# ambicuity/Distributed-LLM-Training-and-Inference-System

Measured on AMD Instinct MI355X. Metric: tokens/sec (node) GPT-7B train, higher is better.
Workload: dtype bf16; 1 GPU; model=gpt-7b, global_batch=16, seq_len=2048, parallelism=dp1, micro_batch=16, grad_accum=1, activation_checkpoint=none, layout=planner

## Files before the change

### llmctl/config/knobs.py

```python

from __future__ import annotations

import contextlib
import dataclasses
import os
from dataclasses import dataclass, fields
from typing import Any, Dict, Iterator, Optional

ENV = "LLMCTL_KNOBS"


@dataclass(frozen=True)
class PerfKnobs:
    gemm64: bool = True
    gemm64_config: int = 304
    fwd64: str = "auto"
    dgrad64: str = "fused"
    wgrad_kernel: bool = True
    swiglu_bwd: str = "side"
    dgrad_transpose: bool = True
    wt_side_stream: bool = True
    fused_fwd: bool = False
    rope_inplace: bool = True
    fused_rope_attn: bool = True
    moe_pad: bool = True
    overlap_optimizer: bool = False
    gemm_tuning: bool = True
    fa_split: int = -1
    fa_prio: int = 1
    fa_nw: int = 4
    dkv: int = 2
    dkv_nwg: int = 0
    async_tp: bool = True
    async_tp_save_full: bool = False
    cp_zigzag: bool = True
    decode_fused: bool = True
    decode_splits: int = 0
    decode_v3: int = 1
    skinny_gemm: str = "auto"
    prefill_swiglu: bool = True
    prefill_fa: bool = True
    prefill_norm_fold: bool = True
    mixed_steps: bool = True
    custom_ar: bool = True
    tp_graphs: bool = True
    async_decode: bool = True
    tp_fused_decode: bool = True

    def as_dict(self) -> Dict[str, Any]:
        return dataclasses.asdict(self)


NATIVE = ("fa_split", "fa_prio", "fa_nw", "dkv", "dkv_nwg", "decode_splits", "decode_v3")
_FIELDS = {f.name: f for f in fields(PerfKnobs)}


def _coerce(name: str, value: Any) -> Any:
    if name not in _FIELDS:
        raise KeyError(f"unknown performance knob {name!r} (known: {', '.join(sorted(_FIELDS))})")
    typ = _FIELDS[name].type
    if typ in ("bool", bool):
        if isinstance(value, str):
            v = value.strip().lower()
            if v not in ("1", "0", "true", "false", "on", "off", "yes", "no"):
                raise ValueError(f"knob {name}: expected a boolean, got {value!r}")
            return v in ("1", "true", "on", "yes")
        return bool(value)
    if typ in ("int", int):
        return int(value)
    return str(value)


def parse_env(spec: Optional[str]) -> Dict[str, Any]:
    out: Dict[str, Any] = {}
    for part in (spec or "").split(","):
        part = part.strip()
        if not part:
            continue
        if "=" not in part:
            raise ValueError(f"{ENV}: expected name=value, got {part!r}")
        k, v = part.split("=", 1)
        out[k.strip()] = _coerce(k.strip(), v.strip())
    return out


_RETIRED_ENV = ("LLMCTL_SIDE_DGRAD", "LLMCTL_DECODE_ATTN_QKV", "LLMCTL_GEMM64_CONFIG", "LLMCTL_SKINNY")
_warned: set = set()


def _warn_retired_env() -> None:
    import warnings

    names = [f"LLMCTL_{n.upper()}" for n in _FIELDS] + list(_RETIRED_ENV)
    for n in names:
        if n in os.environ and n not in _warned:
            _warned.add(n)
            warnings.warn(f"{n} is no longer read (performance switches are knobs now): set "
                          f"{ENV}=\"{n[7:].lower()}=<value>\" or the [perf] config table instead", stacklevel=3)


def resolve(overrides: Optional[Dict[str, Any]] = None, env: bool = True) -> PerfKnobs:
    _warn_retired_env()
    kw = {k: _coerce(k, v) for k, v in (overrides or {}).items()}
    if env:
        kw.update(parse_env(os.environ.get(ENV)))
    return PerfKnobs(**kw)


_ACTIVE: PerfKnobs = resolve()


def knobs() -> PerfKnobs:
    return _ACTIVE


def push_native(k: Optional[PerfKnobs] = None) -> bool:
    k = k or _ACTIVE
    try:
        from llmctl.ops import _lib

        if not _lib.loaded():
            return False
        import torch

        for name in NATIVE:
            torch.ops.llmctl.set_knob(name, int(getattr(k, name)))
        return True
    except Exception:
        return False


def apply(k: PerfKnobs) -> PerfKnobs:
    global _ACTIVE
    _ACTIVE = k
    push_native(k)
    return k


def use(k: PerfKnobs) -> PerfKnobs:
    if k is not _ACTIVE:
        apply(k)
    return k


def with_env(k: PerfKnobs) -> PerfKnobs:
    env = parse_env(os.environ.get(ENV))
    return dataclasses.replace(k, **env) if env else k


def configure(overrides: Optional[Dict[str, Any]] = None) -> PerfKnobs:
    return apply(resolve(overrides))


@contextlib.contextmanager
def override(**kw: Any) -> Iterator[PerfKnobs]:
    old = _ACTIVE
    new = dataclasses.replace(old, **{k: _coerce(k, v) for k, v in kw.items()})
    apply(new)
    try:
        yield new
    finally:
        apply(old)
```

### llmctl/ops/csrc/attn_common.h

```cpp
#pragma once
#include "common.h"

namespace llmctl {
namespace attn {

using bf16x8_t = __attribute__((ext_vector_type(8))) __bf16;
using s4_t = __attribute__((ext_vector_type(4))) short;
using s8_t = __attribute__((ext_vector_type(8))) short;
using f32x16 = __attribute__((ext_vector_type(16))) float;
using lds_s4 = __attribute__((address_space(3))) s4_t;

__device__ __forceinline__ f32x16 mfma32(bf16x8_t a, bf16x8_t b, f32x16 c) {
  return __builtin_amdgcn_mfma_f32_32x32x16_bf16(a, b, c, 0, 0, 0);
}

__device__ __forceinline__ float fast_exp2(float x) { return __builtin_amdgcn_exp2f(x); }

__device__ __forceinline__ float xor32_max(float x) {
  const auto r = __builtin_amdgcn_permlane32_swap(__float_as_uint(x), __float_as_uint(x), false, false);
  return fmaxf(__uint_as_float(r[0]), __uint_as_float(r[1]));
}
__device__ __forceinline__ float xor32_add(float x) {
  const auto r = __builtin_amdgcn_permlane32_swap(__float_as_uint(x), __float_as_uint(x), false, false);
  return __uint_as_float(r[0]) + __uint_as_float(r[1]);
}

__device__ __forceinline__ int acc_row(int i, int h) { return (i & 3) + 8 * (i >> 2) + 4 * h; }

template <int HD>
__device__ __forceinline__ int swz_row(int row) {
  if constexpr (HD == 128) return row & 15;
  else return (row >> 1) & 7;
}
template <int HD>
__device__ __forceinline__ int swz_tr(int row) {
  if constexpr (HD == 128) return ((row & 3) << 2) | ((row >> 2) & 3);
  else return (((row >> 1) & 1) << 2) | ((row >> 2) & 3);
}

template <int HD>
__device__ __forceinline__ int row_off(int row, int chunk) {
  return row * (HD * 2) + ((chunk ^ swz_row<HD>(row)) << 4);
}
template <int HD>
__device__ __forceinline__ int tr_off(int row, int chunk) {
  return row * (HD * 2) + ((chunk ^ swz_tr<HD>(row)) << 4);
}

__device__ __forceinline__ bf16x8_t lds_read_b128(const unsigned char* base, int off) {
  return *reinterpret_cast<const bf16x8_t*>(base + off);
}

template <int HD>
__device__ __forceinline__ bf16x8_t tr_frag(const unsigned char* base, int row0, int col0, int lane) {
  const int h = lane >> 5;
  const int i16 = lane & 15;
  const int q = i16 >> 2, p = i16 & 3;
  const int col = col0 + 16 * ((lane >> 4) & 1) + 4 * p;
  const int chunk = col >> 3;
  const int sub = (col & 7) * 2;
  const int r1 = row0 + 4 * h + q;
  const int r2 = r1 + 8;
  s4_t lo = __builtin_amdgcn_ds_read_tr16_b64_v4i16((lds_s4*)(base + tr_off<HD>(r1, chunk) + sub));
  s4_t hi = __builtin_amdgcn_ds_read_tr16_b64_v4i16((lds_s4*)(base + tr_off<HD>(r2, chunk) + sub));
  s8_t v = {lo[0], lo[1], lo[2], lo[3], hi[0], hi[1], hi[2], hi[3]};
  return __builtin_bit_cast(bf16x8_t, v);
}

template <int HD>
__device__ __forceinline__ void tr_frag_offs(int col0, int lane, int& lo, int& hi) {
  const int h = lane >> 5;
  const int i16 = lane & 15;
  const int q = i16 >> 2, p = i16 & 3;
  const int col = col0 + 16 * ((lane >> 4) & 1) + 4 * p;
  const int chunk = col >> 3;
  const int sub = (col & 7) * 2;
  lo = tr_off<HD>(4 * h + q, chunk) + sub;
  hi = tr_off<HD>(8 + 4 * h + q, chunk) + sub;
}
template <int HD>
__device__ __forceinline__ bf16x8_t tr_frag_at(const unsigned char* base, int row0, int lo, int hi) {
  s4_t a = __builtin_amdgcn_ds_read_tr16_b64_v4i16((lds_s4*)(base + row0 * (HD * 2) + lo));
  s4_t b = __builtin_amdgcn_ds_read_tr16_b64_v4i16((lds_s4*)(base + row0 * (HD * 2) + hi));
  s8_t v = {a[0], a[1], a[2], a[3], b[0], b[1], b[2], b[3]};
  return __builtin_bit_cast(bf16x8_t, v);
}

template <int HD>
__device__ __forceinline__ bf16x8_t tr_frag_nat(const unsigned char* base, int row0, int col0, int lane) {
  const int h = lane >> 5;
  const int i16 = lane & 15;
  const int q = i16 >> 2, p = i16 & 3;
  const int col = col0 + 16 * ((lane >> 4) & 1) + 4 * p;
  const int chunk = col >> 3;
  const int sub = (col & 7) * 2;
  const int r1 = row0 + 8 * h + q;
  const int r2 = r1 + 4;
  s4_t lo = __builtin_amdgcn_ds_read_tr16_b64_v4i16((lds_s4*)(base + tr_off<HD>(r1, chunk) + sub));
  s4_t hi = __builtin_amdgcn_ds_read_tr16_b64_v4i16((lds_s4*)(base + tr_off<HD>(r2, chunk) + sub));
  s8_t v = {lo[0], lo[1], lo[2], lo[3], hi[0], hi[1], hi[2], hi[3]};
  return __builtin_bit_cast(bf16x8_t, v);
}

__device__ __forceinline__ bf16x8_t to_bf16x8(const float* x) {
  bf16x8_t v;
#pragma unroll
  for (int j = 0; j < 8; ++j) v[j] = (__bf16)x[j];
  return v;
}

__device__ __forceinline__ uint4 gload16(const unsigned short* p) { return *reinterpret_cast<const uint4*>(p); }

__device__ __forceinline__ void dma16(const void* g, unsigned lds_byte) {
  asm volatile("s_mov_b32 m0, %1\n\ts_nop 0\n\tglobal_load_lds_dwordx4 %0, off" ::"v"(g), "s"(lds_byte) : "memory");
}
__device__ __forceinline__ void dma4(const void* g, unsigned lds_byte) {
  asm volatile("s_mov_b32 m0, %1\n\ts_nop 0\n\tglobal_load_lds_dword %0, off" ::"v"(g), "s"(lds_byte) : "memory");
}
template <int N>
__device__ __forceinline__ void vm_wait() {
  static_assert(N >= 0 && N <= 15, "vmcnt immediate");
  if constexpr (N == 0) asm volatile("s_waitcnt vmcnt(0)" ::: "memory");
  else if constexpr (N == 5) asm volatile("s_waitcnt vmcnt(5)" ::: "memory");
  else if constexpr (N == 9) asm volatile("s_waitcnt vmcnt(9)" ::: "memory");
  else static_assert(N == 0 || N == 5 || N == 9, "add the immediate");
}
using i32x4_t = __attribute__((ext_vector_type(4))) int;
__device__ __forceinline__ i32x4_t buf_rsrc(const void* base, unsigned num_records) {
  const unsigned long a = (unsigned long)base;
  i32x4_t r;
  r[0] = __builtin_amdgcn_readfirstlane((int)(a & 0xffffffffu));
  r[1] = __builtin_amdgcn_readfirstlane((int)((a >> 32) & 0xffff));
  r[2] = __builtin_amdgcn_readfirstlane((int)num_records);
  r[3] = 0x00020000;
  return r;
}
__device__ __forceinline__ void buf_dma16(i32x4_t rsrc, unsigned voff, unsigned lds_byte) {
  asm volatile("s_mov_b32 m0, %2\n\ts_nop 0\n\tbuffer_load_dwordx4 %0, %1, 0 offen lds" ::"v"(voff), "s"(rsrc),
               "s"(lds_byte)
               : "memory");
}
__device__ __forceinline__ void buf_dma4(i32x4_t rsrc, unsigned voff, unsigned lds_byte) {
  asm volatile("s_mov_b32 m0, %2\n\ts_nop 0\n\tbuffer_load_dword %0, %1, 0 offen lds" ::"v"(voff), "s"(rsrc),
               "s"(lds_byte)
               : "memory");
}
template <int N>
__device__ __forceinline__ void vm_wait_n() {
  static_assert(N >= 0 && N <= 63, "vmcnt immediate");
  asm volatile("s_waitcnt vmcnt(%0)" ::"i"(N) : "memory");
}

__device__ __forceinline__ unsigned lds_addr(const void* p) {
  return __builtin_amdgcn_readfirstlane(
      (unsigned)(uintptr_t)(const __attribute__((address_space(3))) unsigned char*)p);
}

}
}
```

### llmctl/ops/csrc/flash_attn_bwd.hip

```cpp
#include <cstdlib>
#include <map>
#include <mutex>

#include "attn_common.h"

namespace llmctl {
using namespace attn;
namespace {

constexpr float LOG2E = 1.4426950408889634f;
constexpr int KV_KB = 128;
constexpr int KV_QT = 64;
#ifndef LLMCTL_DKV_NBUF
#define LLMCTL_DKV_NBUF 2
#endif
constexpr int KV_NBUF = LLMCTL_DKV_NBUF;
static_assert(KV_NBUF >= 2 && KV_NBUF <= 4, "dK/dV ring depth 2-4");
constexpr int DQ_QB = 128;
constexpr int DQ_KB = 64;

struct BwdArgs {
  const unsigned short *q, *k, *v, *dout;
  const float* lse;
  const float* delta;
  unsigned short *dq, *dk, *dv;
  int B, S, Hq, Hkv;
  long q_sb, q_ss, q_sh, k_sb, k_ss, k_sh, v_sb, v_ss, v_sh, do_sb, do_ss, do_sh;
  float scale, scale_log2;
  const int* doc;
  long dq_st, dk_st, dv_st;
  const float* cos_t;
  const float* sin_t;
  const int* rope_pos;
  int rope_S;
  const unsigned short* o;
  long o_sb, o_ss, o_sh;
  float* delta_w;
  float* rck_w;
  long rc_n;
  unsigned long long* stamps = nullptr;
};

template <int NDB>
__device__ __forceinline__ void dvdk_step(f32x16* dv, f32x16* dk, const bf16x8_t* da, const bf16x8_t* qa, bf16x8_t p,
                                          bf16x8_t ds) {
  if constexpr (NDB == 4) {
    asm volatile(
        "s_nop 1\n\t"
        "v_mfma_f32_32x32x16_bf16 %0, %8, %16, %0\n\t"
        "v_mfma_f32_32x32x16_bf16 %4, %12, %17, %4\n\t"
        "v_mfma_f32_32x32x16_bf16 %1, %9, %16, %1\n\t"
        "v_mfma_f32_32x32x16_bf16 %5, %13, %17, %5\n\t"
        "v_mfma_f32_32x32x16_bf16 %2, %10, %16, %2\n\t"
        "v_mfma_f32_32x32x16_bf16 %6, %14, %17, %6\n\t"
        "v_mfma_f32_32x32x16_bf16 %3, %11, %16, %3\n\t"
        "v_mfma_f32_32x32x16_bf16 %7, %15, %17, %7\n\t"
        "s_nop 11"
        : "+a"(dv[0]), "+a"(dv[1]), "+a"(dv[2]), "+a"(dv[3]), "+a"(dk[0]), "+a"(dk[1]), "+a"(dk[2]), "+a"(dk[3])
        : "v"(da[0]), "v"(da[1]), "v"(da[2]), "v"(da[3]), "v"(qa[0]), "v"(qa[1]), "v"(qa[2]), "v"(qa[3]), "v"(p),
          "v"(ds));
  } else {
    static_assert(NDB == 2, "head_dim 64 or 128");
    asm volatile(
        "s_nop 1\n\t"
        "v_mfma_f32_32x32x16_bf16 %0, %4, %8, %0\n\t"
        "v_mfma_f32_32x32x16_bf16 %2, %6, %9, %2\n\t"
        "v_mfma_f32_32x32x16_bf16 %1, %5, %8, %1\n\t"
        "v_mfma_f32_32x32x16_bf16 %3, %7, %9, %3\n\t"
        "s_nop 11"
        : "+a"(dv[0]), "+a"(dv[1]), "+a"(dk[0]), "+a"(dk[1])
        : "v"(da[0]), "v"(da[1]), "v"(qa[0]), "v"(qa[1]), "v"(p), "v"(ds));
  }
}

__device__ __forceinline__ void store_bf16x4(unsigned short* p, const float* x, float mul) {
  unsigned short w[4];
#pragma unroll
  for (int j = 0; j < 4; ++j) w[j] = f2bf(x[j] * mul);
  *reinterpret_cast<uint2*>(p) =
      make_uint2((unsigned)w[0] | ((unsigned)w[1] << 16), (unsigned)w[2] | ((unsigned)w[3] << 16));
}

template <int HD, typename AccT>
__device__ __forceinline__ void store_row(unsigned short* dst, const AccT* acc, float mul, int hh,
                                          const float* cos_row, const float* sin_row) {
  constexpr int NDB = HD / 32;
  if (cos_row != nullptr) {
    constexpr int HB = NDB / 2;
#pragma unroll
    for (int d = 0; d < HB; ++d)
#pragma unroll
      for (int g = 0; g < 4; ++g) {
        const int c = d * 32 + 8 * g + 4 * hh;
        const float4 cs = *reinterpret_cast<const float4*>(cos_row + c);
        const float4 sn = *reinterpret_cast<const float4*>(sin_row + c);
        const float cv[4] = {cs.x, cs.y, cs.z, cs.w}, sv[4] = {sn.x, sn.y, sn.z, sn.w};
        float lo[4], hi[4];
#pragma unroll
        for (int j = 0; j < 4; ++j) {
          const float x1 = acc[d][4 * g + j], x2 = acc[d + HB][4 * g + j];
          lo[j] = x1 * cv[j] + x2 * sv[j];
          hi[j] = x2 * cv[j] - x1 * sv[j];
        }
        store_bf16x4(dst + c, lo, mul);
        store_bf16x4(dst + c + HD / 2, hi, mul);
      }
    return;
  }
#pragma unroll
  for (int d = 0; d < NDB; ++d)
#pragma unroll
    for (int g = 0; g < 4; ++g) {
      float x[4];
#pragma unroll
      for (int j = 0; j < 4; ++j) x[j] = acc[d][4 * g + j];
      store_bf16x4(dst + d * 32 + 8 * g + 4 * hh, x, mul);
    }
}

template <int HD, bool CAUSAL, bool DOC>
__global__ __launch_bounds__(256, 1) void fa_bwd_dkv_kernel(BwdArgs a) {
  constexpr int NKS = HD / 16;
  constexpr int NDB = HD / 32;
  constexpr int ROWB = HD * 2;
  constexpr int TILE_B = KV_QT * ROWB;
  constexpr int NP = TILE_B / 1024 / 4;
  constexpr int RC_B = KV_QT * 4;
  constexpr int BUF_B = 2 * TILE_B + 4 * RC_B;
  constexpr int NB = KV_NBUF;
  __shared__ __attribute__((aligned(1024))) unsigned char smem[NB * BUF_B];

  const int tid = threadIdx.x;
  const int lane = tid & 63;
  const int wave = __builtin_amdgcn_readfirstlane(tid >> 6);
  const int r = lane & 31, hh = lane >> 5;
  const int nkb = (a.S + KV_KB - 1) / KV_KB;
  const int BH = a.B * a.Hkv;
  int bh, kblk;
  if (BH % 8) {
    bh = blockIdx.x % BH;
    kblk = blockIdx.x / BH;
  } else {
    const int x = blockIdx.x & 7, j = blockIdx.x >> 3;
    bh = x * (BH >> 3) + j / nkb;
    kblk = j % nkb;
  }
  const int b = bh / a.Hkv, hk = bh % a.Hkv;
  const int group = a.Hq / a.Hkv;
  const int k0 = kblk * KV_KB;
  const int wkey0 = k0 + wave * 32;
  const int my_key = wkey0 + r;

#pragma unroll
  for (int i = 0; i < NB * BUF_B / 4096; ++i)
    *reinterpret_cast<uint4*>(smem + i * 4096 + tid * 16) = make_uint4(0, 0, 0, 0);
  if (tid < (NB * BUF_B % 4096) / 16)
    *reinterpret_cast<uint4*>(smem + (NB * BUF_B / 4096) * 4096 + tid * 16) = make_uint4(0, 0, 0, 0);
  __syncthreads();

  const unsigned lds0 = lds_addr(smem);
  bf16x8_t kf[NKS], vf[NKS];
  {
    const int kc = min(my_key, a.S - 1);
    const unsigned short* Kp = a.k + b * a.k_sb + hk * a.k_sh + (long)kc * a.k_ss + 8 * hh;
    const unsigned short* Vp = a.v + b * a.v_sb + hk * a.v_sh + (long)kc * a.v_ss + 8 * hh;
#pragma unroll
    for (int ks = 0; ks < NKS; ++ks) {
      kf[ks] = __builtin_bit_cast(bf16x8_t, gload16(Kp + 16 * ks));
      vf[ks] = __builtin_bit_cast(bf16x8_t, gload16(Vp + 16 * ks));
    }
#pragma unroll
    for (int ks = 0; ks < NKS; ++ks) asm volatile("" ::"v"(kf[ks]), "v"(vf[ks]));
  }

  f32x16 dk[NDB], dv[NDB];
#pragma unroll
  for (int d = 0; d < NDB; ++d)
#pragma unroll
    for (int i = 0; i < 16; ++i) dk[d][i] = dv[d][i] = 0.f;

  const int q_start = CAUSAL ? k0 : 0;
  int q_end = a.S;
  if constexpr (DOC) {
    const int* ds = a.doc + (long)b * a.S;
    int lo = min(k0 + KV_KB, a.S), hi = a.S;
    while (lo < hi) {
      const int mid = (lo + hi) >> 1;
      if (ds[mid] > k0 + KV_KB - 1) hi = mid;
      else lo = mid + 1;
    }
    q_end = __builtin_amdgcn_readfirstlane(lo);
  }
  const int nq = q_end > q_start ? (q_end - q_start + KV_QT - 1) / KV_QT : 0;
  const int ntiles = group * nq;
  unsigned vq[NP], vd[NP];
#pragma unroll
  for (int i = 0; i < NP; ++i) {
    const int byte = (i * 4 + wave) * 1024 + lane * 16;
    const int row = byte / ROWB;
    const int lch = ((byte % ROWB) >> 4) ^ swz_tr<HD>(row);
    vq[i] = (unsigned)((row * a.q_ss + lch * 8) * 2);
    vd[i] = (unsigned)((row * a.do_ss + lch * 8) * 2);
  }
  const float* rc_src = a.rck_w + (wave == 1 ? a.rc_n : 0);
  const unsigned rc_off =
      (DOC && wave == 2) ? lane * 4
                         : (unsigned)((32 * (lane >> 5) + 8 * ((lane >> 2) & 3) + 4 * ((lane >> 4) & 1) + (lane & 3)) * 4);
  int iq0 = q_start;
  const unsigned short* qh = a.q + b * a.q_sb + (long)(hk * group) * a.q_sh;
  const unsigned short* dh = a.dout + b * a.do_sb + (long)(hk * group) * a.do_sh;
  const float* rh = rc_src + ((long)b * a.Hq + hk * group) * a.S;
  const unsigned short* qc = qh + (long)q_start * a.q_ss;
  const unsigned short* dc = dh + (long)q_start * a.do_ss;
  const long q_step = (long)KV_QT * a.q_ss, d_step = (long)KV_QT * a.do_ss;
  constexpr int PT = 2 * NP + 1;
  auto issue = [&](auto slot_c) __attribute__((always_inline)) {
    constexpr int SLC = decltype(slot_c)::value;
    const int nr = min(KV_QT, a.S - iq0);
    i32x4_t rq = buf_rsrc(qc, (unsigned)(((nr - 1) * a.q_ss + HD) * 2));
    i32x4_t rd = buf_rsrc(dc, (unsigned)(((nr - 1) * a.do_ss + HD) * 2));
    i32x4_t rr = (DOC && wave == 2) ? buf_rsrc(a.doc + (long)b * a.S + iq0, (unsigned)(nr * 4))
                                    : buf_rsrc(rh + iq0, (unsigned)(nr * 4));
    asm volatile("s_nop 4" : "+s"(rq), "+s"(rd), "+s"(rr));
    const unsigned slot = lds0 + (unsigned)(SLC * BUF_B);
#pragma unroll
    for (int i = 0; i < NP; ++i) {
      buf_dma16(rq, vq[i], slot + (i * 4 + wave) * 1024);
      buf_dma16(rd, vd[i], slot + TILE_B + (i * 4 + wave) * 1024);
    }
    buf_dma4(rr, rc_off, slot + 2 * TILE_B + wave * RC_B);
    iq0 += KV_QT;
    qc += q_step;
    dc += d_step;
    if (iq0 >= q_end) {
      iq0 = q_start;
      qh += a.q_sh;
      dh += a.do_sh;
      rh += a.S;
      qc = qh + (long)q_start * a.q_ss;
      dc = dh + (long)q_start * a.do_ss;
    }
  };

  if (ntiles > 0) issue(std::integral_constant<int, 0>{});
  if constexpr (NB >= 3)
    if (ntiles > 1) issue(std::integral_constant<int, 1>{});
  if constexpr (NB >= 4)
    if (ntiles > 2) issue(std::integral_constant<int, 2>{});
  int qi = 0;
  auto step = [&](auto slot_c, int t) __attribute__((always_inline)) {
    constexpr int SL = decltype(slot_c)::value;
    const int younger = min(NB - 2, ntiles - 1 - t);
    if (NB >= 4 && younger >= 2) vm_wait_n<(NB >= 4 ? 2 * PT : 0)>();
    else if (NB >= 3 && younger >= 1) vm_wait_n<(NB >= 3 ? PT : 0)>();
    else vm_wait_n<0>();
    __builtin_amdgcn_s_barrier();
    if (t + NB - 1 < ntiles) issue(std::integral_constant<int, (SL + NB - 1) % NB>{});
    const int q0 = q_start + qi * KV_QT;
    if (++qi == nq) qi = 0;
    if (CAUSAL && wkey0 > q0 + KV_QT - 1) return;
    const bool need_mask = DOC || (CAUSAL && wkey0 + 31 > q0) || (q0 + KV_QT > a.S) || (wkey0 + 31 >= a.S);
    const unsigned char* Qs = smem + SL * BUF_B;
    const unsigned char* Ds = Qs + TILE_B;
    const float* lse_s = reinterpret_cast<const float*>(Ds + TILE_B);
    const float* del_s = lse_s + KV_QT;
    const int* doc_s = reinterpret_cast<const int*>(del_s + KV_QT);

#pragma unroll
    for (int h = 0; h < 2; ++h) {
      f32x16 s, dp;
      {
        bf16x8_t qa[NKS], da[NKS];
#pragma unroll
        for (int ks = 0; ks < NKS; ++ks) {
          qa[ks] = lds_read_b128(Qs, tr_off<HD>(32 * h + r, 2 * ks + hh));
          da[ks] = lds_read_b128(Ds, tr_off<HD>(32 * h + r, 2 * ks + hh));
        }
        s = *reinterpret_cast<const f32x16*>(lse_s + 32 * h + 16 * hh);
        dp = *reinterpret_cast<const f32x16*>(del_s + 32 * h + 16 * hh);
#pragma unroll
        for (int ks = 0; ks < NKS; ++ks) {
          s = mfma32(qa[ks], kf[ks], s);
          dp = mfma32(da[ks], vf[ks], dp);
        }
      }
      __builtin_amdgcn_sched_barrier(0);
      bf16x8_t dfr[NDB], qfr[NDB];
      if constexpr (CAUSAL) {
#pragma unroll
        for (int d = 0; d < NDB; ++d) {
          dfr[d] = tr_frag<HD>(Ds, 32 * h, d * 32, lane);
          qfr[d] = tr_frag<HD>(Qs, 32 * h, d * 32, lane);
        }
      }
      __builtin_amdgcn_sched_barrier(0);
      if (need_mask) {
#pragma unroll
        for (int gq = 0; gq < 4; ++gq) {
          const int row0 = 32 * h + 8 * gq + 4 * hh;
          int sv[4] = {0, 0, 0, 0};
          if constexpr (DOC) {
            const int4 s4 = *reinterpret_cast<const int4*>(doc_s + row0);
            sv[0] = s4.x; sv[1] = s4.y; sv[2] = s4.z; sv[3] = s4.w;
          }
#pragma unroll
          for (int j = 0; j < 4; ++j) {
            const int qq = q0 + row0 + j;
            bool ok = qq < a.S && my_key < a.S;
            if constexpr (CAUSAL) ok = ok && my_key <= qq;
            if constexpr (DOC) ok = ok && my_key >= sv[j];
            s[4 * gq + j] = ok ? s[4 * gq + j] : -INFINITY;
          }
        }
      }
      float p[16], dsv[16];
#pragma unroll
      for (int i = 0; i < 16; ++i) {
        const float pv = fast_exp2(s[i] * a.scale_log2);
        p[i] = pv;
        dsv[i] = pv * dp[i];
      }
      bf16x8_t pb[2], sb[2];
      pb[0] = to_bf16x8(p);
      pb[1] = to_bf16x8(p + 8);
      sb[0] = to_bf16x8(dsv);
      sb[1] = to_bf16x8(dsv + 8);
      if constexpr (!CAUSAL) {
#pragma unroll
        for (int d = 0; d < NDB; ++d) {
          dfr[d] = tr_frag<HD>(Ds, 32 * h, d * 32, lane);
          qfr[d] = tr_frag<HD>(Qs, 32 * h, d * 32, lane);
        }
      }
      bf16x8_t dfr1[NDB], qfr1[NDB];
#pragma unroll
      for (int d = 0; d < NDB; ++d) {
        dfr1[d] = tr_frag<HD>(Ds, 32 * h + 16, d * 32, lane);
        qfr1[d] = tr_frag<HD>(Qs, 32 * h + 16, d * 32, lane);
      }
      dvdk_step<NDB>(dv, dk, dfr, qfr, pb[0], sb[0]);
      dvdk_step<NDB>(dv, dk, dfr1, qfr1, pb[1], sb[1]);
    }
  };
  for (int t = 0; t < ntiles; t += NB) {
    step(std::integral_constant<int, 0>{}, t);
    if (t + 1 < ntiles) step(std::integral_constant<int, 1>{}, t + 1);
    if constexpr (NB >= 3)
      if (t + 2 < ntiles) step(std::integral_constant<int, 2 % NB>{}, t + 2);
    if constexpr (NB >= 4)
      if (t + 3 < ntiles) step(std::integral_constant<int, 3 % NB>{}, t + 3);
  }
#pragma unroll
  for (int d = 0; d < NDB; ++d) asm volatile("s_nop 7\n\ts_nop 7" : "+a"(dk[d]), "+a"(dv[d]));
  if (my_key < a.S) {
    const long tok = (long)b * a.S + my_key;
    unsigned short* dkp = a.dk + tok * a.dk_st + (long)hk * HD;
    unsigned short* dvp = a.dv + tok * a.dv_st + (long)hk * HD;
    const float *cr = nullptr, *sr = nullptr;
    if (a.cos_t != nullptr) {
      const long p = a.rope_pos ? (long)a.rope_pos[tok] : tok % a.rope_S;
      cr = a.cos_t + p * (HD / 2);
      sr = a.sin_t + p * (HD / 2);
    }
    store_row<HD>(dkp, dk, a.scale, hh, cr, sr);
    store_row<HD>(dvp, dv, 1.f, hh, nullptr, nullptr);
  }
}

using s2_t = __attribute__((ext_vector_type(2))) unsigned int;

__device__ __forceinline__ bf16x8_t words8(unsigned w0, unsigned w1, unsigned w2, unsigned w3) {
  using u4 = __attribute__((ext_vector_type(4))) unsigned;
  return __builtin_bit_cast(bf16x8_t, u4{w0, w1, w2, w3});
}

__device__ __forceinline__ void mfma_v(f32x16& acc, bf16x8_t a, bf16x8_t b) {
  asm volatile("v_mfma_f32_32x32x16_bf16 %0, %1, %2, %0" : "+v"(acc) : "v"(a), "a"(b) : "memory");
}

__device__ __forceinline__ void x_step(f32x16& acc_s, f32x16& acc_d, bf16x8_t a_s, bf16x8_t b_s, bf16x8_t a_d,
                                       bf16x8_t b_d, float s0, float s1, float d0, float d1, float c, unsigned& pw,
                                       unsigned& dw) {
  float t0, t1, p0, p1;
  asm volatile(
      "v_mul_f32 %[t0], %[c], %[s0]\n\t"
      "v_mul_f32 %[t1], %[c], %[s1]\n\t"
      "v_mfma_f32_32x32x16_bf16 %[as], %[xs], %[ys], %[as]\n\t"
      "v_exp_f32 %[p0], %[t0]\n\t"
      "v_exp_f32 %[p1], %[t1]\n\t"
      "v_mfma_f32_32x32x16_bf16 %[ad], %[xd], %[yd], %[ad]\n\t"
      "v_mul_f32 %[t0], %[p0], %[d0]\n\t"
      "v_mul_f32 %[t1], %[p1], %[d1]\n\t"
      "v_cvt_pk_bf16_f32 %[pw], %[p0], %[p1]\n\t"
      "v_cvt_pk_bf16_f32 %[dw], %[t0], %[t1]"
      : [as] "+v"(acc_s), [ad] "+v"(acc_d), [t0] "=&v"(t0), [t1] "=&v"(t1), [p0] "=&v"(p0), [p1] "=&v"(p1),
        [pw] "=&v"(pw), [dw] "=&v"(dw)
      : [xs] "v"(a_s), [ys] "a"(b_s), [xd] "v"(a_d), [yd] "a"(b_d), [s0] "v"(s0), [s1] "v"(s1), [d0] "v"(d0),
        [d1] "v"(d1), [c] "s"(c)
      : "memory");
}

__device__ __forceinline__ void y_step(f32x16& dv, f32x16& dk, bf16x8_t da, bf16x8_t qa, bf16x8_t p, bf16x8_t ds,
                                       float s0, float s1, float d0, float d1, float c, unsigned& pw, unsigned& dw) {
  float t0, t1, p0, p1;
  asm volatile(
      "v_mul_f32 %[t0], %[c], %[s0]\n\t"
      "v_mul_f32 %[t1], %[c], %[s1]\n\t"
      "v_mfma_f32_32x32x16_bf16 %[dv], %[da], %[p], %[dv]\n\t"
      "v_exp_f32 %[p0], %[t0]\n\t"
      "v_exp_f32 %[p1], %[t1]\n\t"
      "v_mfma_f32_32x32x16_bf16 %[dk], %[qa], %[ds], %[dk]\n\t"
      "v_mul_f32 %[t0], %[p0], %[d0]\n\t"
      "v_mul_f32 %[t1], %[p1], %[d1]\n\t"
      "v_cvt_pk_bf16_f32 %[pw], %[p0], %[p1]\n\t"
      "v_cvt_pk_bf16_f32 %[dw], %[t0], %[t1]"
      : [dv] "+a"(dv), [dk] "+a"(dk), [t0] "=&v"(t0), [t1] "=&v"(t1), [p0] "=&v"(p0), [p1] "=&v"(p1),
        [pw] "=&v"(pw), [dw] "=&v"(dw)
      : [da] "v"(da), [qa] "v"(qa), [p] "v"(p), [ds] "v"(ds), [s0] "v"(s0), [s1] "v"(s1), [d0] "v"(d0),
        [d1] "v"(d1), [c] "s"(c)
      : "memory");
}

__device__ __forceinline__ f32x16 acc_copy(const f32x16& acc) {
  f32x16 out = acc;
  asm volatile("" : "+v"(out)::"memory");
  return out;
}
__device__ __forceinline__ void acc_zero(f32x16& acc) {
  const bf16x8_t z = {};
  asm volatile("s_nop 2\n\tv_mfma_f32_32x32x16_bf16 %0, %1, %1, 0" : "+a"(acc) : "v"(z));
}

__device__ __forceinline__ void z_step(f32x16& dv, f32x16& dk, bf16x8_t da, bf16x8_t qa, bf16x8_t p, bf16x8_t ds) {
  asm volatile(
      "v_mfma_f32_32x32x16_bf16 %[dv], %[da], %[p], %[dv]\n\t"
      "v_mfma_f32_32x32x16_bf16 %[dk], %[qa], %[ds], %[dk]"
      : [dv] "+a"(dv), [dk] "+a"(dk)
      : [da] "v"(da), [qa] "v"(qa), [p] "v"(p), [ds] "v"(ds)
      : "memory");
}

template <int HD, bool CAUSAL, bool DOC, bool STAMP = false>
__global__ __launch_bounds__(256, 1) void fa_bwd_dkv_pipe_kernel(BwdArgs a) {
  static_assert(HD == 128 && CAUSAL, "pipelined dK/dV kernel: causal, head_dim 128");
  constexpr int NKS = HD / 16;
  constexpr int NDB = HD / 32;
  constexpr int ROWB = HD * 2;
  constexpr int TILE_B = KV_QT * ROWB;
  constexpr int NP = TILE_B / 1024 / 4;
  constexpr int RC_B = KV_QT * 4;
  constexpr int BUF_B = 2 * TILE_B + 4 * RC_B;
  __shared__ __attribute__((aligned(1024))) unsigned char smem[2 * BUF_B];

  const int tid = threadIdx.x;
  const int lane = tid & 63;
  const int wave = __builtin_amdgcn_readfirstlane(tid >> 6);
  const int r = lane & 31, hh = lane >> 5;
  auto stamp = [&](int i) __attribute__((always_inline)) {
    if constexpr (STAMP) {
      if (tid == 0) a.stamps[blockIdx.x * 8 + i] = __builtin_amdgcn_s_memrealtime();
    }
  };
  stamp(0);
  if constexpr (STAMP) {
    if (tid == 0)
      a.stamps[blockIdx.x * 8 + 1] = (unsigned long long)(unsigned)__builtin_amdgcn_s_getreg(63492) |
                                     ((unsigned long long)(unsigned)__builtin_amdgcn_s_getreg(63508) << 32);
  }
  const int nkb = (a.S + KV_KB - 1) / KV_KB;
  const int BH = a.B * a.Hkv;
  int bh, kblk;
  if (BH % 8) {
    bh = blockIdx.x % BH;
    kblk = blockIdx.x / BH;
  } else {
    const int x = blockIdx.x & 7, j = blockIdx.x >> 3;
    bh = x * (BH >> 3) + j / nkb;
    kblk = j % nkb;
  }
  const int b = bh / a.Hkv, hk = bh % a.Hkv;
  const int group = a.Hq / a.Hkv;
  const int k0 = kblk * KV_KB;
  const int wkey0 = k0 + wave * 32;
  const int my_key = wkey0 + r;

  if (a.S % KV_QT) {
#pragma unroll
    for (int i = 0; i < 2 * BUF_B / 4096; ++i)
      *reinterpret_cast<uint4*>(smem + i * 4096 + tid * 16) = make_uint4(0, 0, 0, 0);
    if (tid < (2 * BUF_B % 4096) / 16)
      *reinterpret_cast<uint4*>(smem + (2 * BUF_B / 4096) * 4096 + tid * 16) = make_uint4(0, 0, 0, 0);
    __syncthreads();
  }

  const unsigned lds0 = lds_addr(smem);

  f32x16 dk[NDB], dv[NDB];
#pragma unroll
  for (int d = 0; d < NDB; ++d)
#pragma unroll
    for (int i = 0; i < 16; ++i) dk[d][i] = dv[d][i] = 0.f;

  const int q_start = CAUSAL ? k0 : 0;
  int q_end = a.S;
  if constexpr (DOC) {
    const int* ds = a.doc + (long)b * a.S;
    int lo = min(k0 + KV_KB, a.S), hi = a.S;
    while (lo < hi) {
      const int mid = (lo + hi) >> 1;
      if (ds[mid] > k0 + KV_KB - 1) hi = mid;
      else lo = mid + 1;
    }
    q_end = __builtin_amdgcn_readfirstlane(lo);
  }
  const int nq = q_end > q_start ? (q_end - q_start + KV_QT - 1) / KV_QT : 0;
  const int ntiles = group * nq;
  unsigned vq[NP], vd[NP];
#pragma unroll
  for (int i = 0; i < NP; ++i) {
    const int byte = (i * 4 + wave) * 1024 + lane * 16;
    const int row = byte / ROWB;
    const int lch = ((byte % ROWB) >> 4) ^ swz_tr<HD>(row);
    vq[i] = (unsigned)((row * a.q_ss + lch * 8) * 2);
    vd[i] = (unsigned)((row * a.do_ss + lch * 8) * 2);
  }
  const float* rc_src = a.rck_w + (wave == 1 ? a.rc_n : 0);
  const unsigned rc_off =
      (DOC && wave == 2) ? lane * 4
                         : (unsigned)((32 * (lane >> 5) + 8 * ((lane >> 2) & 3) + 4 * ((lane >> 4) & 1) + (lane & 3)) * 4);
  int iq0 = q_start;
  const unsigned short* qh = a.q + b * a.q_sb + (long)(hk * group) * a.q_sh;
  const unsigned short* dh = a.dout + b * a.do_sb + (long)(hk * group) * a.do_sh;
  const float* rh = rc_src + ((long)b * a.Hq + hk * group) * a.S;
  const unsigned short* qc = qh + (long)q_start * a.q_ss;
  const unsigned short* dc = dh + (long)q_start * a.do_ss;
  const long q_step = (long)KV_QT * a.q_ss, d_step = (long)KV_QT * a.do_ss;
  auto issue = [&](auto slot_c) __attribute__((always_inline)) {
    constexpr int SLC = decltype(slot_c)::value;
    const int nr = min(KV_QT, a.S - iq0);
    i32x4_t rq = buf_rsrc(qc, (unsigned)(((nr - 1) * a.q_ss + HD) * 2));
    i32x4_t rd = buf_rsrc(dc, (unsigned)(((nr - 1) * a.do_ss + HD) * 2));
    i32x4_t rr = (DOC && wave == 2) ? buf_rsrc(a.doc + (long)b * a.S + iq0, (unsigned)(nr * 4))
                                    : buf_rsrc(rh + iq0, (unsigned)(nr * 4));
    asm volatile("s_nop 4" : "+s"(rq), "+s"(rd), "+s"(rr));
    const unsigned slot = lds0 + (unsigned)(SLC * BUF_B);
#pragma unroll
    for (int i = 0; i < NP; ++i) {
      buf_dma16(rq, vq[i], slot + (i * 4 + wave) * 1024);
      buf_dma16(rd, vd[i], slot + TILE_B + (i * 4 + wave) * 1024);
    }
    buf_dma4(rr, rc_off, slot + 2 * TILE_B + wave * RC_B);
    iq0 += KV_QT;
    qc += q_step;
    dc += d_step;
    if (iq0 >= q_end) {
      iq0 = q_start;
      qh += a.q_sh;
      dh += a.do_sh;
      rh += a.S;
      qc = qh + (long)q_start * a.q_ss;
      dc = dh + (long)q_start * a.do_ss;
    }
  };

  const float c = a.scale_log2;
  auto apply_mask = [&](f32x16& s, int h, int q0, const int* doc_s) __attribute__((always_inline)) {
#pragma unroll
    for (int gq = 0; gq < 4; ++gq) {
      const int row0 = 32 * h + 8 * gq + 4 * hh;
      int sv[4] = {0, 0, 0, 0};
      if constexpr (DOC) {
        const int4 s4 = *reinterpret_cast<const int4*>(doc_s + row0);
        sv[0] = s4.x; sv[1] = s4.y; sv[2] = s4.z; sv[3] = s4.w;
      }
#pragma unroll
      for (int j = 0; j < 4; ++j) {
        const int qq = q0 + row0 + j;
        bool ok = qq < a.S && my_key < a.S;
        if constexpr (CAUSAL) ok = ok && my_key <= qq;
        if constexpr (DOC) ok = ok && my_key >= sv[j];
        s[4 * gq + j] = ok ? s[4 * gq + j] : -INFINITY;
      }
    }
  };

  if (ntiles > 0) issue(std::integral_constant<int, 0>{});
  bf16x8_t kf[NKS], vf[NKS];
  {
    const int kc = min(my_key, a.S - 1);
    const unsigned short* Kp = a.k + b * a.k_sb + hk * a.k_sh + (long)kc * a.k_ss + 8 * hh;
    const unsigned short* Vp = a.v + b * a.v_sb + hk * a.v_sh + (long)kc * a.v_ss + 8 * hh;
#pragma unroll
    for (int ks = 0; ks < NKS; ++ks) {
      asm volatile("global_load_dwordx4 %0, %1, off" : "=a"(kf[ks]) : "v"(Kp + 16 * ks) : "memory");
      asm volatile("global_load_dwordx4 %0, %1, off" : "=a"(vf[ks]) : "v"(Vp + 16 * ks) : "memory");
    }
  }
  vm_wait_n<0>();
  __builtin_amdgcn_s_barrier();
  stamp(2);
  if (ntiles > 1) issue(std::integral_constant<int, 1>{});
  int qi = 0;
  auto tile = [&](auto slot_c, int t) __attribute__((always_inline)) {
    constexpr int SL = decltype(slot_c)::value;
    const int q0 = q_start + qi * KV_QT;
    if (++qi == nq) qi = 0;
    const bool live = !(CAUSAL && wkey0 > q0 + KV_QT - 1);
    const unsigned char* Qs = smem + SL * BUF_B;
    const unsigned char* Ds = Qs + TILE_B;
    const float* lse_s = reinterpret_cast<const float*>(Ds + TILE_B);
    const float* del_s = lse_s + KV_QT;
    const int* doc_s = reinterpret_cast<const int*>(del_s + KV_QT);
    if (!live) return;
    f32x16 s0 = *reinterpret_cast<const f32x16*>(lse_s + 16 * hh);
    f32x16 p0 = *reinterpret_cast<const f32x16*>(del_s + 16 * hh);
    bf16x8_t qa[NKS], da[NKS];
#pragma unroll
    for (int ks = 0; ks < NKS; ++ks) {
      qa[ks] = lds_read_b128(Qs, tr_off<HD>(r, 2 * ks + hh));
      da[ks] = lds_read_b128(Ds, tr_off<HD>(r, 2 * ks + hh));
    }
    const bool need_mask = DOC || (CAUSAL && wkey0 + 31 > q0) || (q0 + KV_QT > a.S) || (wkey0 + 31 >= a.S);
#pragma unroll
    for (int ks = 0; ks < NKS; ++ks) {
      mfma_v(s0, qa[ks], kf[ks]);
      mfma_v(p0, da[ks], vf[ks]);
    }
    f32x16 s1 = *reinterpret_cast<const f32x16*>(lse_s + 32 + 16 * hh);
    f32x16 p1 = *reinterpret_cast<const f32x16*>(del_s + 32 + 16 * hh);
#pragma unroll
    for (int ks = 0; ks < NKS; ++ks) {
      qa[ks] = lds_read_b128(Qs, tr_off<HD>(32 + r, 2 * ks + hh));
      da[ks] = lds_read_b128(Ds, tr_off<HD>(32 + r, 2 * ks + hh));
    }
    if (need_mask) apply_mask(s0, 0, q0, doc_s);
    unsigned pw0[8], dw0[8];
    bf16x8_t td[2][NDB], tq[2][NDB];
#pragma unroll
    for (int ks = 0; ks < NKS; ++ks) {
      x_step(s1, p1, qa[ks], kf[ks], da[ks], vf[ks], s0[2 * ks], s0[2 * ks + 1], p0[2 * ks], p0[2 * ks + 1], c, pw0[ks],
             dw0[ks]);
      const int st = ks >> 2, d = ks & 3;
      td[st][d] = tr_frag<HD>(Ds, 16 * st, d * 32, lane);
      tq[st][d] = tr_frag<HD>(Qs, 16 * st, d * 32, lane);
    }
    if (need_mask) apply_mask(s1, 1, q0, doc_s);
    unsigned pw1[8], dw1[8];
    bf16x8_t cd[2][NDB], cq[2][NDB];
#pragma unroll
    for (int st = 0; st < 2; ++st) {
      const bf16x8_t pb = words8(pw0[4 * st], pw0[4 * st + 1], pw0[4 * st + 2], pw0[4 * st + 3]);
      const bf16x8_t sb = words8(dw0[4 * st], dw0[4 * st + 1], dw0[4 * st + 2], dw0[4 * st + 3]);
#pragma unroll
      for (int d = 0; d < NDB; ++d) {
        const int i = 4 * st + d;
        y_step(dv[d], dk[d], td[st][d], tq[st][d], pb, sb, s1[2 * i], s1[2 * i + 1], p1[2 * i], p1[2 * i + 1], c,
               pw1[i], dw1[i]);
        cd[st][d] = tr_frag<HD>(Ds, 32 + 16 * st, d * 32, lane);
        cq[st][d] = tr_frag<HD>(Qs, 32 + 16 * st, d * 32, lane);
      }
    }
#pragma unroll
    for (int st = 0; st < 2; ++st) {
      const bf16x8_t pb = words8(pw1[4 * st], pw1[4 * st + 1], pw1[4 * st + 2], pw1[4 * st + 3]);
      const bf16x8_t sb = words8(dw1[4 * st], dw1[4 * st + 1], dw1[4 * st + 2], dw1[4 * st + 3]);
#pragma unroll
      for (int d = 0; d < NDB; ++d) z_step(dv[d], dk[d], cd[st][d], cq[st][d], pb, sb);
    }
  };
  auto advance = [&](auto slot_c, int t) __attribute__((always_inline)) {
    constexpr int SL = decltype(slot_c)::value;
    asm volatile("s_waitcnt lgkmcnt(0)" ::: "memory");
    vm_wait_n<0>();
    __builtin_amdgcn_s_barrier();
    if (t + 2 < ntiles) issue(std::integral_constant<int, SL>{});
  };
  for (int t = 0; t < ntiles; t += 2) {
    tile(std::integral_constant<int, 0>{}, t);
    advance(std::integral_constant<int, 0>{}, t);
    if (t + 1 < ntiles) {
      tile(std::integral_constant<int, 1>{}, t + 1);
      advance(std::integral_constant<int, 1>{}, t + 1);
    }
  }
  stamp(3);
#pragma unroll
  for (int d = 0; d < NDB; ++d) asm volatile("s_nop 7\n\ts_nop 7" : "+a"(dk[d]), "+a"(dv[d]));
  if (my_key < a.S) {
    const long tok = (long)b * a.S + my_key;
    unsigned short* dkp = a.dk + tok * a.dk_st + (long)hk * HD;
    unsigned short* dvp = a.dv + tok * a.dv_st + (long)hk * HD;
    const float *cr = nullptr, *sr = nullptr;
    if (a.cos_t != nullptr) {
      const long p = a.rope_pos ? (long)a.rope_pos[tok] : tok % a.rope_S;
      cr = a.cos_t + p * (HD / 2);
      sr = a.sin_t + p * (HD / 2);
    }
    store_row<HD>(dkp, dk, a.scale, hh, cr, sr);
    store_row<HD>(dvp, dv, 1.f, hh, nullptr, nullptr);
  }
  if constexpr (STAMP) {
    asm volatile("s_waitcnt vmcnt(0)" ::: "memory");
    __syncthreads();
    stamp(4);
    if (tid == 0) a.stamps[blockIdx.x * 8 + 5] = (unsigned long long)ntiles;
  }
}

template <bool STAMP>
__global__ __launch_bounds__(256, 1) void fa_bwd_dkv_persist_kernel(BwdArgs a, int* __restrict__ wq) {
  constexpr int HD = 128;
  constexpr int NKS = HD / 16;
  constexpr int NDB = HD / 32;
  constexpr int ROWB = HD * 2;
  constexpr int TILE_B = KV_QT * ROWB;
  constexpr int NP = TILE_B / 1024 / 4;
  constexpr int RC_B = KV_QT * 4;
  constexpr int BUF_B = 2 * TILE_B + 4 * RC_B;
  __shared__ __attribute__((aligned(1024))) unsigned char smem[2 * BUF_B + 64];
  int* item_w = reinterpret_cast<int*>(smem + 2 * BUF_B);

  const int tid = threadIdx.x;
  const int lane = tid & 63;
  const int wave = __builtin_amdgcn_readfirstlane(tid >> 6);
  const int r = lane & 31, hh = lane >> 5;
  const int nkb = a.S / KV_KB;
  const int BH = a.B * a.Hkv;
  const bool per_xcd = BH % 8 == 0;
  const int xq = per_xcd ? (int)(blockIdx.x & 7) : 0;
  const int n_items = (per_xcd ? BH / 8 : BH) * nkb;
  const int bh_base = per_xcd ? xq * (BH / 8) : 0;
  const int group = a.Hq / a.Hkv;
  auto pop = [&]() __attribute__((always_inline)) -> int {
    const int j = __hip_atomic_fetch_add(wq + xq, 1, __ATOMIC_RELAXED, __HIP_MEMORY_SCOPE_AGENT);
    return j < n_items ? j : -1;
  };
  if (tid == 0) {
    const int i0 = pop();
    item_w[1] = i0;
    item_w[2] = i0 >= 0 ? pop() : -1;
  }
  __syncthreads();
  int cur = __builtin_amdgcn_readfirstlane(item_w[1]);
  int nxt = __builtin_amdgcn_readfirstlane(item_w[2]);
  if (cur < 0) return;

  const unsigned lds0 = lds_addr(smem);
  unsigned vq[NP], vd[NP];
#pragma unroll
  for (int i = 0; i < NP; ++i) {
    const int byte = (i * 4 + wave) * 1024 + lane * 16;
    const int row = byte / ROWB;
    const int lch = ((byte % ROWB) >> 4) ^ swz_tr<HD>(row);
    vq[i] = (unsigned)((row * a.q_ss + lch * 8) * 2);
    vd[i] = (unsigned)((row * a.do_ss + lch * 8) * 2);
  }
  const float* rc_src = a.rck_w + (wave == 1 ? a.rc_n : 0);
  const unsigned rc_off =
      (unsigned)((32 * (lane >> 5) + 8 * ((lane >> 2) & 3) + 4 * ((lane >> 4) & 1) + (lane & 3)) * 4);

  int iss = cur, iq0 = 0, iq_start = 0, ig = 0;
  const unsigned short *qh = nullptr, *dh = nullptr;
  const float* rh = nullptr;
  bool look_pending = false;
  int n_switch = 0;
  int pend0 = -1, pend1 = -1, npend = 0;
  auto iss_begin = [&](int item) __attribute__((always_inline)) {
    const int bh = bh_base + item / nkb, kb = item % nkb;
    const int bb = bh / a.Hkv, hkk = bh % a.Hkv;
    iq_start = kb * KV_KB;
    iq0 = iq_start;
    ig = 0;
    qh = a.q + bb * a.q_sb + (long)(hkk * group) * a.q_sh;
    dh = a.dout + bb * a.do_sb + (long)(hkk * group) * a.do_sh;
    rh = rc_src + ((long)bb * a.Hq + hkk * group) * a.S;
  };
  iss_begin(cur);
  auto issue = [&](auto slot_c) __attribute__((always_inline)) {
    constexpr int SLC = decltype(slot_c)::value;
    i32x4_t rq = buf_rsrc(qh + (long)iq0 * a.q_ss, (unsigned)(((KV_QT - 1) * a.q_ss + HD) * 2));
    i32x4_t rd = buf_rsrc(dh + (long)iq0 * a.do_ss, (unsigned)(((KV_QT - 1) * a.do_ss + HD) * 2));
    i32x4_t rr = buf_rsrc(rh + iq0, (unsigned)(KV_QT * 4));
    asm volatile("s_nop 4" : "+s"(rq), "+s"(rd), "+s"(rr));
    const unsigned slot = lds0 + (unsigned)(SLC * BUF_B);
#pragma unroll
    for (int i = 0; i < NP; ++i) {
      buf_dma16(rq, vq[i], slot + (i * 4 + wave) * 1024);
      buf_dma16(rd, vd[i], slot + TILE_B + (i * 4 + wave) * 1024);
    }
    buf_dma4(rr, rc_off, slot + 2 * TILE_B + wave * RC_B);
    iq0 += KV_QT;
    if (iq0 >= a.S) {
      if (++ig < group) {
        iq0 = iq_start;
        qh += a.q_sh;
        dh += a.do_sh;
        rh += a.S;
      } else {
        iss = nxt;
        if (iss >= 0) {
          iss_begin(iss);
          if (tid == 0) item_w[3 + (n_switch & 1)] = pop();
          look_pending = true;
          ++n_switch;
        }
        if (npend == 0) pend0 = iss;
        else pend1 = iss;
        ++npend;
      }
    }
  };

  bf16x8_t kf[NKS], vf[NKS];
  auto load_kv = [&](int item) __attribute__((always_inline)) {
    const int bh = bh_base + item / nkb, kb = item % nkb;
    const int bb = bh / a.Hkv, hkk = bh % a.Hkv;
    const int key = kb * KV_KB + wave * 32 + r;
    const unsigned short* Kp = a.k + bb * a.k_sb + hkk * a.k_sh + (long)key * a.k_ss + 8 * hh;
    const unsigned short* Vp = a.v + bb * a.v_sb + hkk * a.v_sh + (long)key * a.v_ss + 8 * hh;
#pragma unroll
    for (int ks = 0; ks < NKS; ++ks) {
      asm volatile("global_load_dwordx4 %0, %1, off" : "+a"(kf[ks]) : "v"(Kp + 16 * ks) : "memory");
      asm volatile("global_load_dwordx4 %0, %1, off" : "+a"(vf[ks]) : "v"(Vp + 16 * ks) : "memory");
    }
  };

  issue(std::integral_constant<int, 0>{});
  load_kv(cur);
  asm volatile("s_waitcnt vmcnt(0)"
               : "+a"(kf[0]), "+a"(kf[1]), "+a"(kf[2]), "+a"(kf[3]), "+a"(kf[4]), "+a"(kf[5]), "+a"(kf[6]),
                 "+a"(kf[7]), "+a"(vf[0]), "+a"(vf[1]), "+a"(vf[2]), "+a"(vf[3]), "+a"(vf[4]), "+a"(vf[5]),
                 "+a"(vf[6]), "+a"(vf[7])
               :
               : "memory");
  __builtin_amdgcn_s_barrier();
  issue(std::integral_constant<int, 1>{});
  f32x16 dk[NDB], dv[NDB];
#pragma unroll
  for (int d = 0; d < NDB; ++d) {
    const bf16x8_t z = {};
    asm volatile("s_nop 2\n\tv_mfma_f32_32x32x16_bf16 %0, %1, %1, 0" : "=a"(dk[d]) : "v"(z));
    asm volatile("v_mfma_f32_32x32x16_bf16 %0, %1, %1, 0" : "=a"(dv[d]) : "v"(z));
  }
  const float c = a.scale_log2;

  int n_done = 0;
  auto stamp = [&](int k) __attribute__((always_inline)) {
    if constexpr (STAMP) {
      if (tid == 0 && n_done < 64)
        a.stamps[(blockIdx.x * 64 + n_done) * 4 + k] = k == 3 ? (unsigned long long)cur : __builtin_amdgcn_s_memrealtime();
    }
  };
  for (;;) {
    stamp(0);
    stamp(3);
    const int bh = bh_base + cur / nkb, kb = cur % nkb;
    const int b = bh / a.Hkv, hk = bh % a.Hkv;
    const int k0 = kb * KV_KB;
    const int wkey0 = k0 + wave * 32;
    const int my_key = wkey0 + r;
    const int ntiles = group * ((a.S - k0) / KV_QT);
    int q0 = k0;
    auto apply_mask = [&](f32x16& s, int h) __attribute__((always_inline)) {
#pragma unroll
      for (int gq = 0; gq < 4; ++gq) {
        const int row0 = q0 + 32 * h + 8 * gq + 4 * hh;
#pragma unroll
        for (int j = 0; j < 4; ++j) s[4 * gq + j] = my_key <= row0 + j ? s[4 * gq + j] : -INFINITY;
      }
    };
    auto tile = [&](auto slot_c) __attribute__((always_inline)) {
      constexpr int SL = decltype(slot_c)::value;
      const bool live = !(wkey0 > q0 + KV_QT - 1);
      if (!live) return;
      const unsigned char* Qs = smem + SL * BUF_B;
      const unsigned char* Ds = Qs + TILE_B;
      const float* lse_s = reinterpret_cast<const float*>(Ds + TILE_B);
      const float* del_s = lse_s + KV_QT;
      const bool need_mask = wkey0 + 31 > q0;
      f32x16 s0 = *reinterpret_cast<const f32x16*>(lse_s + 16 * hh);
      f32x16 p0 = *reinterpret_cast<const f32x16*>(del_s + 16 * hh);
      bf16x8_t qa[NKS], da[NKS];
#pragma unroll
      for (int ks = 0; ks < NKS; ++ks) {
        qa[ks] = lds_read_b128(Qs, tr_off<HD>(r, 2 * ks + hh));
        da[ks] = lds_read_b128(Ds, tr_off<HD>(r, 2 * ks + hh));
      }
      f32x16 s1 = *reinterpret_cast<const f32x16*>(lse_s + 32 + 16 * hh);
      f32x16 p1 = *reinterpret_cast<const f32x16*>(del_s + 32 + 16 * hh);
      bf16x8_t qb[NKS], db[NKS];
#pragma unroll
      for (int ks = 0; ks < NKS; ++ks) {
        mfma_v(s0, qa[ks], kf[ks]);
        qb[ks] = lds_read_b128(Qs, tr_off<HD>(32 + r, 2 * ks + hh));
        mfma_v(p0, da[ks], vf[ks]);
        db[ks] = lds_read_b128(Ds, tr_off<HD>(32 + r, 2 * ks + hh));
      }
      if (need_mask) apply_mask(s0, 0);
      unsigned pw0[8], dw0[8];
      bf16x8_t td[2][NDB], tq[2][NDB];
#pragma unroll
      for (int ks = 0; ks < NKS; ++ks) {
        x_step(s1, p1, qb[ks], kf[ks], db[ks], vf[ks], s0[2 * ks], s0[2 * ks + 1], p0[2 * ks], p0[2 * ks + 1], c,
               pw0[ks], dw0[ks]);
        const int st = ks >> 2, d = ks & 3;
        td[st][d] = tr_frag<HD>(Ds, 16 * st, d * 32, lane);
        tq[st][d] = tr_frag<HD>(Qs, 16 * st, d * 32, lane);
      }
      if (need_mask) apply_mask(s1, 1);
      unsigned pw1[8], dw1[8];
      bf16x8_t cd[2][NDB], cq[2][NDB];
#pragma unroll
      for (int st = 0; st < 2; ++st) {
        const bf16x8_t pb = words8(pw0[4 * st], pw0[4 * st + 1], pw0[4 * st + 2], pw0[4 * st + 3]);
        const bf16x8_t sb = words8(dw0[4 * st], dw0[4 * st + 1], dw0[4 * st + 2], dw0[4 * st + 3]);
#pragma unroll
        for (int d = 0; d < NDB; ++d) {
          const int i = 4 * st + d;
          y_step(dv[d], dk[d], td[st][d], tq[st][d], pb, sb, s1[2 * i], s1[2 * i + 1], p1[2 * i], p1[2 * i + 1], c,
                 pw1[i], dw1[i]);
          cd[st][d] = tr_frag<HD>(Ds, 32 + 16 * st, d * 32, lane);
          cq[st][d] = tr_frag<HD>(Qs, 32 + 16 * st, d * 32, lane);
        }
      }
#pragma unroll
      for (int st = 0; st < 2; ++st) {
        const bf16x8_t pb = words8(pw1[4 * st], pw1[4 * st + 1], pw1[4 * st + 2], pw1[4 * st + 3]);
        const bf16x8_t sb = words8(dw1[4 * st], dw1[4 * st + 1], dw1[4 * st + 2], dw1[4 * st + 3]);
#pragma unroll
        for (int d = 0; d < NDB; ++d) z_step(dv[d], dk[d], cd[st][d], cq[st][d], pb, sb);
      }
    };
    auto advance = [&](auto slot_c) __attribute__((always_inline)) {
      constexpr int SL = decltype(slot_c)::value;
      asm volatile("s_waitcnt lgkmcnt(0)" ::: "memory");
      vm_wait_n<0>();
      __builtin_amdgcn_s_barrier();
      if (look_pending) {
        nxt = __builtin_amdgcn_readfirstlane(item_w[3 + ((n_switch - 1) & 1)]);
        look_pending = false;
      }
      if (iss >= 0) issue(std::integral_constant<int, SL>{});
      q0 += KV_QT;
      if (q0 >= a.S) q0 = k0;
    };
    for (int t = 0; t < ntiles; t += 2) {
      tile(std::integral_constant<int, 0>{});
      advance(std::integral_constant<int, 0>{});
      tile(std::integral_constant<int, 1>{});
      advance(std::integral_constant<int, 1>{});
    }
    stamp(1);
    {
      const long tok = (long)b * a.S + my_key;
      unsigned short* dkp = a.dk + tok * a.dk_st + (long)hk * HD;
      unsigned short* dvp = a.dv + tok * a.dv_st + (long)hk * HD;
      const bool rope = a.cos_t != nullptr;
      f32x4 cs[NDB / 2][4], sn[NDB / 2][4];
      if (rope) {
        const long p = a.rope_pos ? (long)a.rope_pos[tok] : tok % a.rope_S;
        const float* cr = a.cos_t + p * (HD / 2);
        const float* sr = a.sin_t + p * (HD / 2);
#pragma unroll
        for (int d = 0; d < NDB / 2; ++d)
#pragma unroll
          for (int g = 0; g < 4; ++g) {
            const int col = d * 32 + 8 * g + 4 * hh;
            cs[d][g] = *reinterpret_cast<const f32x4*>(cr + col);
            sn[d][g] = *reinterpret_cast<const f32x4*>(sr + col);
          }
      }
#pragma unroll
      for (int d = 0; d < NDB; ++d) asm volatile("s_nop 7\n\ts_nop 7" : "+a"(dk[d]), "+a"(dv[d]));
      auto st8 = [&](unsigned short* p, const float* x, float mul) __attribute__((always_inline)) {
        s2_t w;
        w[0] = (unsigned)f2bf(x[0] * mul) | ((unsigned)f2bf(x[1] * mul) << 16);
        w[1] = (unsigned)f2bf(x[2] * mul) | ((unsigned)f2bf(x[3] * mul) << 16);
        asm volatile("global_store_dwordx2 %0, %1, off" ::"v"(p), "v"(w) : "memory");
      };
#pragma unroll
      for (int d = 0; d < NDB / 2; ++d) {
        const f32x16 x1 = acc_copy(dk[d]), x2 = acc_copy(dk[d + NDB / 2]);
        acc_zero(dk[d]);
        acc_zero(dk[d + NDB / 2]);
#pragma unroll
        for (int g = 0; g < 4; ++g) {
          const int col = d * 32 + 8 * g + 4 * hh;
          float lo[4], hi[4];
#pragma unroll
          for (int j = 0; j < 4; ++j) {
            const float c1 = rope ? cs[d][g][j] : 1.f, s1 = rope ? sn[d][g][j] : 0.f;
            lo[j] = x1[4 * g + j] * c1 + x2[4 * g + j] * s1;
            hi[j] = x2[4 * g + j] * c1 - x1[4 * g + j] * s1;
          }
          st8(dkp + col, lo, a.scale);
          st8(dkp + col + HD / 2, hi, a.scale);
        }
      }
#pragma unroll
      for (int d = 0; d < NDB; ++d) {
        const f32x16 x = acc_copy(dv[d]);
        acc_zero(dv[d]);
#pragma unroll
        for (int g = 0; g < 4; ++g) {
          float y[4];
#pragma unroll
          for (int j = 0; j < 4; ++j) y[j] = x[4 * g + j];
          st8(dvp + d * 32 + 8 * g + 4 * hh, y, 1.f);
        }
      }
      load_kv(pend0 >= 0 ? pend0 : cur);
      asm volatile("s_waitcnt vmcnt(0)"
                   : "+a"(kf[0]), "+a"(kf[1]), "+a"(kf[2]), "+a"(kf[3]), "+a"(kf[4]), "+a"(kf[5]), "+a"(kf[6]),
                     "+a"(kf[7]), "+a"(vf[0]), "+a"(vf[1]), "+a"(vf[2]), "+a"(vf[3]), "+a"(vf[4]), "+a"(vf[5]),
                     "+a"(vf[6]), "+a"(vf[7])
                   :
                   : "memory");
    }
    stamp(2);
    ++n_done;
    if (pend0 < 0) break;
    cur = pend0;
    pend0 = pend1;
    pend1 = -1;
    --npend;
  }
}

template <int HD, bool CAUSAL, bool DOC>
__global__ __launch_bounds__(256, 2) void fa_bwd_dq_kernel(BwdArgs a) {
  constexpr int NKS = HD / 16;
  constexpr int NDB = HD / 32;
  constexpr int ROWB = HD * 2;
  constexpr int TILE = DQ_KB * ROWB;
  constexpr int PPW = TILE / 1024 / 4;
  constexpr int SLOT = 2 * TILE;
  __shared__ __attribute__((aligned(1024))) unsigned char smem[2 * SLOT];

  const int tid = threadIdx.x;
  const int lane = tid & 63;
  const int wave = __builtin_amdgcn_readfirstlane(tid >> 6);
  const int r = lane & 31, hh = lane >> 5;
  const int nqb = (a.S + DQ_QB - 1) / DQ_QB;
  const int BH = a.B * a.Hq;
  int bh, qi;
  if (BH % 8) {
    bh = blockIdx.x % BH;
    qi = blockIdx.x / BH;
  } else {
    const int x = blockIdx.x & 7, j = blockIdx.x >> 3;
    bh = x * (BH >> 3) + j / nqb;
    qi = j % nqb;
  }
  const int qblk = nqb - 1 - qi;
  const int b = bh / a.Hq, hq = bh % a.Hq;
  const int hk = hq / (a.Hq / a.Hkv);
  const int q_row0 = qblk * DQ_QB + wave * 32;
  const int my_q = q_row0 + r;
  const int qc = min(my_q, a.S - 1);

  const unsigned short* Kp = a.k + b * a.k_sb + hk * a.k_sh;
  const unsigned short* Vp = a.v + b * a.v_sb + hk * a.v_sh;

#pragma unroll
  for (int i = 0; i < 2 * SLOT / 4096; ++i)
    *reinterpret_cast<uint4*>(smem + i * 4096 + tid * 16) = make_uint4(0, 0, 0, 0);

  bf16x8_t qf[NKS], df[NKS];
  {
    const unsigned short* Qp = a.q + b * a.q_sb + hq * a.q_sh + (long)qc * a.q_ss + 8 * hh;
    const unsigned short* Dp = a.dout + b * a.do_sb + hq * a.do_sh + (long)qc * a.do_ss + 8 * hh;
#pragma unroll
    for (int ks = 0; ks < NKS; ++ks) {
      qf[ks] = __builtin_bit_cast(bf16x8_t, gload16(Qp + 16 * ks));
      df[ks] = __builtin_bit_cast(bf16x8_t, gload16(Dp + 16 * ks));
    }
  }
  const long rc = ((long)b * a.Hq + hq) * a.S + qc;
  const float nlse2 = -a.lse[rc] * LOG2E;
  float dlt;
  if (a.o != nullptr) {
    const unsigned short* Op = a.o + b * a.o_sb + hq * a.o_sh + (long)qc * a.o_ss + 8 * hh;
    float acc = 0.f;
#pragma unroll
    for (int ks = 0; ks < NKS; ++ks) {
      const bf16x8_t of = __builtin_bit_cast(bf16x8_t, gload16(Op + 16 * ks));
#pragma unroll
      for (int j = 0; j < 8; ++j) acc += (float)of[j] * (float)df[ks][j];
    }
    dlt = xor32_add(acc);
    if (hh == 0 && my_q < a.S) a.delta_w[rc] = dlt;
  } else {
    dlt = a.delta[rc];
  }
  if (hh == 0 && my_q < a.S) {
    a.rck_w[rc] = -a.lse[rc] / a.scale;
    a.rck_w[a.rc_n + rc] = -dlt;
  }
#pragma unroll
  for (int ks = 0; ks < NKS; ++ks) asm volatile("" ::"v"(qf[ks]), "v"(df[ks]));
  asm volatile("" ::"v"(nlse2), "v"(dlt));

  f32x16 dq[NDB];
#pragma unroll
  for (int d = 0; d < NDB; ++d)
#pragma unroll
    for (int i = 0; i < 16; ++i) dq[d][i] = 0.f;

  const int kv_end = CAUSAL ? min(a.S, qblk * DQ_QB + DQ_QB) : a.S;
  const int ntiles = (kv_end + DQ_KB - 1) / DQ_KB;
  int my_start = 0, w_min = 0, w_max = 0, t0 = 0;
  if constexpr (DOC) {
    const int* ds = a.doc + (long)b * a.S;
    my_start = ds[qc];
    w_min = __builtin_amdgcn_readfirstlane(ds[min(q_row0, a.S - 1)]);
    w_max = __builtin_amdgcn_readfirstlane(ds[min(q_row0 + 31, a.S - 1)]);
    t0 = __builtin_amdgcn_readfirstlane(ds[min(qblk * DQ_QB, a.S - 1)]) / DQ_KB;
  }
  const int key_hi = CAUSAL ? qc : a.S - 1;
  int klo[NDB], khi[NDB];
#pragma unroll
  for (int d = 0; d < NDB; ++d) tr_frag_offs<HD>(d * 32, lane, klo[d], khi[d]);
  int kro[NKS], vro[NKS];
#pragma unroll
  for (int ks = 0; ks < NKS; ++ks) {
    kro[ks] = tr_off<HD>(r, 2 * ks + hh);
    vro[ks] = row_off<HD>(r, 2 * ks + hh);
  }

  unsigned vk[PPW], vv[PPW];
#pragma unroll
  for (int i = 0; i < PPW; ++i) {
    const int byte = (i * 4 + wave) * 1024 + lane * 16;
    const int row = byte / ROWB, pch = (byte % ROWB) >> 4;
    vk[i] = (unsigned)((row * a.k_ss + ((pch ^ swz_tr<HD>(row)) << 3)) * 2);
    vv[i] = (unsigned)((row * a.v_ss + ((pch ^ swz_row<HD>(row)) << 3)) * 2);
  }
  const unsigned lds0 = lds_addr(smem);
  int ik0 = t0 * DQ_KB;
  const unsigned short* kc = Kp + (long)ik0 * a.k_ss;
  const unsigned short* vc = Vp + (long)ik0 * a.v_ss;
  const long k_step = (long)DQ_KB * a.k_ss, v_step = (long)DQ_KB * a.v_ss;
  auto issue = [&](auto slot_c) __attribute__((always_inline)) {
    constexpr int SLC = decltype(slot_c)::value;
    const int nk = min(DQ_KB, a.S - ik0);
    i32x4_t rk = buf_rsrc(kc, (unsigned)(((nk - 1) * a.k_ss + HD) * 2));
    i32x4_t rv = buf_rsrc(vc, (unsigned)(((nk - 1) * a.v_ss + HD) * 2));
    asm volatile("s_nop 4" : "+s"(rk), "+s"(rv));
    const unsigned slot = lds0 + (unsigned)(SLC * SLOT) + wave * 1024;
#pragma unroll
    for (int i = 0; i < PPW; ++i) {
      buf_dma16(rk, vk[i], slot + i * 4096);
      buf_dma16(rv, vv[i], slot + TILE + i * 4096);
    }
    ik0 += DQ_KB;
    kc += k_step;
    vc += v_step;
  };

  auto tile = [&](bool need_mask, const unsigned char* Ks, const unsigned char* Vs, int kv0)
                  __attribute__((always_inline)) {
#pragma unroll
    for (int kb = 0; kb < 2; ++kb) {
      f32x16 s, dp;
#pragma unroll
      for (int i = 0; i < 16; ++i) s[i] = dp[i] = 0.f;
#pragma unroll
      for (int ks = 0; ks < NKS; ++ks) {
        s = mfma32(lds_read_b128(Ks, kb * 32 * (HD * 2) + kro[ks]), qf[ks], s);
        dp = mfma32(lds_read_b128(Vs, kb * 32 * (HD * 2) + vro[ks]), df[ks], dp);
      }
      if (need_mask) {
#pragma unroll
        for (int i = 0; i < 16; ++i) {
          const int key = kv0 + kb * 32 + acc_row(i, hh);
          bool ok = key <= key_hi;
          if constexpr (DOC) ok = ok && key >= my_start;
          s[i] = ok ? s[i] : -INFINITY;
        }
      }
      float dsv[16];
#pragma unroll
      for (int i = 0; i < 16; ++i) dsv[i] = fast_exp2(__builtin_fmaf(s[i], a.scale_log2, nlse2)) * (dp[i] - dlt);
#pragma unroll
      for (int st = 0; st < 2; ++st) {
        const bf16x8_t sbf = to_bf16x8(dsv + 8 * st);
#pragma unroll
        for (int d = 0; d < NDB; ++d) dq[d] = mfma32(tr_frag_at<HD>(Ks, kb * 32 + 16 * st, klo[d], khi[d]), sbf, dq[d]);
      }
    }
  };

  __syncthreads();
  auto step = [&](auto slot_c, int t) __attribute__((always_inline)) {
    constexpr int SL = decltype(slot_c)::value;
    vm_wait_n<0>();
    __builtin_amdgcn_s_barrier();
    if (t + 1 < ntiles) issue(std::integral_constant<int, 1 - SL>{});
    const int kv0 = t * DQ_KB;
    bool live = true;
    if constexpr (CAUSAL) live = kv0 <= q_row0 + 31;
    if constexpr (DOC) live = live && kv0 + DQ_KB > w_min;
    if (live) {
      const bool need_mask =
          (CAUSAL && kv0 + DQ_KB - 1 > q_row0) || (kv0 + DQ_KB > a.S) || (DOC && kv0 < w_max);
      tile(need_mask, smem + SL * SLOT, smem + SL * SLOT + TILE, kv0);
    }
  };
  if (t0 < ntiles) issue(std::integral_constant<int, 0>{});
  for (int t = t0; t < ntiles; t += 2) {
    step(std::integral_constant<int, 0>{}, t);
    if (t + 1 < ntiles) step(std::integral_constant<int, 1>{}, t + 1);
  }
  if (my_q < a.S) {
    const long tok = (long)b * a.S + my_q;
    const float *cr = nullptr, *sr = nullptr;
    if (a.cos_t != nullptr) {
      const long p = a.rope_pos ? (long)a.rope_pos[tok] : tok % a.rope_S;
      cr = a.cos_t + p * (HD / 2);
      sr = a.sin_t + p * (HD / 2);
    }
    store_row<HD>(a.dq + tok * a.dq_st + (long)hq * HD, dq, a.scale, hh, cr, sr);
  }
}

int dkv_mode() {
  const int64_t m = knob("dkv", 2);
  return (m >= 0 && m <= 2) ? (int)m : 2;
}

int* dkv_queue(hipStream_t s) {
  static std::mutex mu;
  static std::map<std::pair<int, hipStream_t>, int*> bufs;
  int dev = 0;
  LLMCTL_HIP_CHECK(hipGetDevice(&dev));
  std::lock_guard<std::mutex> lk(mu);
  int*& q = bufs[{dev, s}];
  if (q == nullptr) LLMCTL_HIP_CHECK(hipMalloc(&q, 64 * sizeof(int)));
  return q;
}

template <int HD, bool CAUSAL, bool DOC>
void launch_bwd(const BwdArgs& a, hipStream_t s, bool do_dq, bool do_dkv, int dkv_impl) {
  if (do_dq) {
    const int nqb = (a.S + DQ_QB - 1) / DQ_QB;
    hipLaunchKernelGGL((fa_bwd_dq_kernel<HD, CAUSAL, DOC>), dim3((unsigned)(a.B * a.Hq * nqb)), dim3(256), 0, s, a);
  }
  if (do_dkv) {
    const int nkb = (a.S + KV_KB - 1) / KV_KB;
    const dim3 grid((unsigned)(a.B * a.Hkv * nkb));
    if constexpr (HD == 128 && CAUSAL) {
      if (dkv_impl == 2 && a.stamps != nullptr) {
        hipLaunchKernelGGL((fa_bwd_dkv_pipe_kernel<HD, CAUSAL, DOC, true>), grid, dim3(256), 0, s, a);
        return;
      }
      if constexpr (!DOC) {
        if (a.S % KV_KB == 0 && (dkv_impl == 3 || dkv_impl == 4 || (dkv_impl < 0 && dkv_mode() == 2))) {
          int* wq = dkv_queue(s);
          LLMCTL_HIP_CHECK(hipMemsetAsync(wq, 0, 8 * sizeof(int), s));
          int nwg = std::min<long>((long)num_cus(), (long)a.B * a.Hkv * nkb);
          const int min_wg = ((long)a.B * a.Hkv) % 8 == 0 ? 8 : 1;
          if (const int64_t e = knob("dkv_nwg", 0); e > 0) nwg = std::max<int>(min_wg, std::min<int>(nwg, (int)e));
          nwg = std::max(nwg, min_wg);
          if (a.stamps != nullptr)
            hipLaunchKernelGGL(fa_bwd_dkv_persist_kernel<true>, dim3((unsigned)nwg), dim3(256), 0, s, a, wq);
          else
            hipLaunchKernelGGL(fa_bwd_dkv_persist_kernel<false>, dim3((unsigned)nwg), dim3(256), 0, s, a, wq);
          return;
        }
      }
      if (dkv_impl == 1 || dkv_impl == 3 || (dkv_impl < 0 && dkv_mode() >= 1)) {
        hipLaunchKernelGGL((fa_bwd_dkv_pipe_kernel<HD, CAUSAL, DOC>), grid, dim3(256), 0, s, a);
        return;
      }
    }
    hipLaunchKernelGGL((fa_bwd_dkv_kernel<HD, CAUSAL, DOC>), grid, dim3(256), 0, s, a);
  }
}

void dispatch_bwd(const BwdArgs& a, int D, bool causal, bool doc, hipStream_t s, bool do_dq = true,
                  bool do_dkv = true, int dkv_impl = -1) {
  if (doc) {
    if (D == 128) launch_bwd<128, true, true>(a, s, do_dq, do_dkv, dkv_impl);
    else launch_bwd<64, true, true>(a, s, do_dq, do_dkv, dkv_impl);
  } else if (D == 128) {
    if (causal) launch_bwd<128, true, false>(a, s, do_dq, do_dkv, dkv_impl);
    else launch_bwd<128, false, false>(a, s, do_dq, do_dkv, dkv_impl);
  } else {
    if (causal) launch_bwd<64, true, false>(a, s, do_dq, do_dkv, dkv_impl);
    else launch_bwd<64, false, false>(a, s, do_dq, do_dkv, dkv_impl);
  }
}

BwdArgs make_args(const at::Tensor& dout, const at::Tensor& q, const at::Tensor& k, const at::Tensor& v,
                  const at::Tensor& lse, const at::Tensor& delta, at::Tensor& dq, at::Tensor& dk, at::Tensor& dv,
                  double scale) {
  return BwdArgs{bf_ptr(q), bf_ptr(k), bf_ptr(v), bf_ptr(dout), lse.data_ptr<float>(), delta.data_ptr<float>(),
                 bf_mut(dq), bf_mut(dk), bf_mut(dv), (int)q.size(0), (int)q.size(1), (int)q.size(2),
                 (int)k.size(2), q.stride(0), q.stride(1), q.stride(2), k.stride(0), k.stride(1), k.stride(2),
                 v.stride(0), v.stride(1), v.stride(2), dout.stride(0), dout.stride(1), dout.stride(2),
                 (float)scale, (float)(scale * 1.4426950408889634), nullptr,
                 (long)dq.size(2) * dq.size(3), (long)dk.size(2) * dk.size(3), (long)dv.size(2) * dv.size(3),
                 nullptr, nullptr, nullptr, 0, nullptr, 0, 0, 0, nullptr, nullptr, 0};
}

at::Tensor row_consts(BwdArgs& a, const at::Tensor& lse) {
  auto rck = at::empty({2 * lse.numel()}, lse.options());
  a.rck_w = rck.data_ptr<float>();
  a.rc_n = lse.numel();
  return rck;
}

}

std::tuple<at::Tensor, at::Tensor, at::Tensor> flash_attn_bwd(const at::Tensor& dout, const at::Tensor& q,
                                                              const at::Tensor& k, const at::Tensor& v,
                                                              const at::Tensor& o, const at::Tensor& lse,
                                                              double scale, bool causal,
                                                              const c10::optional<at::Tensor>& doc_start) {
  LLMCTL_CHECK(q.dim() == 4 && k.dim() == 4 && v.dim() == 4 && o.dim() == 4 && dout.dim() == 4,
               "flash_attn_bwd: [B,S,H,D] tensors");
  const int B = q.size(0), S = q.size(1), Hq = q.size(2), D = q.size(3);
  const int Hkv = k.size(2);
  LLMCTL_CHECK(D == 64 || D == 128, "head_dim must be 64 or 128");
  LLMCTL_CHECK(Hkv > 0 && Hq % Hkv == 0, "Hq must be a multiple of Hkv");
  LLMCTL_CHECK(dout.sizes() == q.sizes() && o.sizes() == q.sizes() && k.sizes() == v.sizes() && k.size(0) == B &&
                   k.size(1) == S && k.size(3) == D,
               "shape mismatch");
  LLMCTL_CHECK(lse.scalar_type() == at::kFloat && lse.is_contiguous() && lse.numel() == (long)B * Hq * S,
               "lse must be contiguous fp32 [B,Hq,S]");
  for (const at::Tensor* t : {&dout, &q, &k, &v, &o})
    LLMCTL_CHECK(t->is_cuda() && t->scalar_type() == at::kBFloat16 && t->stride(3) == 1 && t->stride(0) % 8 == 0 &&
                     t->stride(1) % 8 == 0 && t->stride(2) % 8 == 0 &&
                     (reinterpret_cast<uintptr_t>(t->data_ptr()) & 15) == 0,
                 "flash_attn_bwd: bf16, d-contiguous, 16-B aligned rows");
  const c10::DeviceGuard g(q.device());
  auto delta = at::empty({B, Hq, S}, q.options().dtype(at::kFloat));
  auto dq = at::empty({B, S, Hq, D}, q.options());
  auto dk = at::empty({B, S, Hkv, D}, q.options());
  auto dv = at::empty({B, S, Hkv, D}, q.options());
  if ((long)B * S * Hq == 0) return {dq, dk, dv};
  auto s = stream();
  BwdArgs a = make_args(dout, q, k, v, lse, delta, dq, dk, dv, scale);
  a.o = bf_ptr(o);
  a.o_sb = o.stride(0);
  a.o_ss = o.stride(1);
  a.o_sh = o.stride(2);
  a.delta_w = delta.data_ptr<float>();
  auto rck = row_consts(a, lse);
  bool doc = false;
  if (doc_start.has_value() && doc_start->defined()) {
    const at::Tensor& ds = *doc_start;
    LLMCTL_CHECK(causal && ds.is_cuda() && ds.scalar_type() == at::kInt && ds.is_contiguous() && ds.dim() == 2 &&
                     ds.size(0) == B && ds.size(1) == S,
                 "flash_attn_bwd: doc_start must be contiguous int32 [B,S] (causal)");
    a.doc = ds.data_ptr<int>();
    doc = true;
  }
  dispatch_bwd(a, D, causal, doc, s);
  return {dq, dk, dv};
}

at::Tensor flash_attn_bwd_qkv(const at::Tensor& dout, const at::Tensor& q, const at::Tensor& k, const at::Tensor& v,
                              const at::Tensor& o, const at::Tensor& lse, double scale, bool causal,
                              const c10::optional<at::Tensor>& doc_start, const at::Tensor& cos_t,
                              const at::Tensor& sin_t, const c10::optional<at::Tensor>& positions, int64_t seq_len) {
  LLMCTL_CHECK(q.dim() == 4 && k.dim() == 4 && v.dim() == 4 && o.dim() == 4 && dout.dim() == 4,
               "flash_attn_bwd_qkv: [B,S,H,D] tensors");
  const int B = q.size(0), S = q.size(1), Hq = q.size(2), D = q.size(3);
  const int Hkv = k.size(2);
  LLMCTL_CHECK(D == 64 || D == 128, "head_dim must be 64 or 128");
  LLMCTL_CHECK(Hkv > 0 && Hq % Hkv == 0, "Hq must be a multiple of Hkv");
  LLMCTL_CHECK(dout.sizes() == q.sizes() && o.sizes() == q.sizes() && k.sizes() == v.sizes() && k.size(0) == B &&
                   k.size(1) == S && k.size(3) == D,
               "shape mismatch");
  LLMCTL_CHECK(lse.scalar_type() == at::kFloat && lse.is_contiguous() && lse.numel() == (long)B * Hq * S,
               "lse must be contiguous fp32 [B,Hq,S]");
  for (const at::Tensor* t : {&dout, &q, &k, &v, &o})
    LLMCTL_CHECK(t->is_cuda() && t->scalar_type() == at::kBFloat16 && t->stride(3) == 1 && t->stride(0) % 8 == 0 &&
                     t->stride(1) % 8 == 0 && t->stride(2) % 8 == 0 &&
                     (reinterpret_cast<uintptr_t>(t->data_ptr()) & 15) == 0,
                 "flash_attn_bwd_qkv: bf16, d-contiguous, 16-B aligned rows");
  LLMCTL_CHECK(cos_t.is_cuda() && sin_t.is_cuda() && cos_t.scalar_type() == at::kFloat &&
                   sin_t.scalar_type() == at::kFloat && cos_t.is_contiguous() && sin_t.is_contiguous() &&
                   cos_t.dim() == 2 && cos_t.size(1) == D / 2 && sin_t.sizes() == cos_t.sizes(),
               "flash_attn_bwd_qkv: cos/sin fp32 contiguous [P, D/2]");
  const bool has_pos = positions.has_value() && positions->defined();
  if (has_pos) {
    LLMCTL_CHECK(positions->is_cuda() && positions->scalar_type() == at::kInt && positions->is_contiguous() &&
                     positions->numel() == (long)B * S,
                 "flash_attn_bwd_qkv: positions int32 [B*S]");
  } else {
    LLMCTL_CHECK(seq_len > 0 && seq_len <= cos_t.size(0), "flash_attn_bwd_qkv: seq_len within the tables");
  }
  const c10::DeviceGuard g(q.device());
  const long W = (long)(Hq + 2 * Hkv) * D;
  auto dqkv = at::empty({(long)B * S, W}, q.options());
  if ((long)B * S * Hq == 0) return dqkv;
  auto delta = at::empty({B, Hq, S}, q.options().dtype(at::kFloat));
  auto s = stream();
  unsigned short* base = bf_mut(dqkv);
  BwdArgs a{bf_ptr(q), bf_ptr(k), bf_ptr(v), bf_ptr(dout), lse.data_ptr<float>(), delta.data_ptr<float>(),
            base, base + (long)Hq * D, base + (long)(Hq + Hkv) * D, B, S, Hq, Hkv,
            q.stride(0), q.stride(1), q.stride(2), k.stride(0), k.stride(1), k.stride(2),
            v.stride(0), v.stride(1), v.stride(2), dout.stride(0), dout.stride(1), dout.stride(2),
            (float)scale, (float)(scale * 1.4426950408889634), nullptr, W, W, W,
            cos_t.data_ptr<float>(), sin_t.data_ptr<float>(), has_pos ? positions->data_ptr<int>() : nullptr,
            (int)(has_pos ? 1 : seq_len), bf_ptr(o), o.stride(0), o.stride(1), o.stride(2),
            delta.data_ptr<float>(), nullptr, 0};
  auto rck = row_consts(a, lse);
  bool doc = false;
  if (doc_start.has_value() && doc_start->defined()) {
    const at::Tensor& ds = *doc_start;
    LLMCTL_CHECK(causal && ds.is_cuda() && ds.scalar_type() == at::kInt && ds.is_contiguous() && ds.dim() == 2 &&
                     ds.size(0) == B && ds.size(1) == S,
                 "flash_attn_bwd_qkv: doc_start must be contiguous int32 [B,S] (causal)");
    a.doc = ds.data_ptr<int>();
    doc = true;
  }
  dispatch_bwd(a, D, causal, doc, s);
  return dqkv;
}

void fa_bwd_ablate(const at::Tensor& dout, const at::Tensor& q, const at::Tensor& k, const at::Tensor& v,
                   const at::Tensor& delta, const at::Tensor& lse, at::Tensor& dq, at::Tensor& dk, at::Tensor& dv,
                   int64_t abl) {
  const int D = q.size(3);
  LLMCTL_CHECK(D == 64 || D == 128, "fa_bwd_ablate: head_dim 64 or 128");
  LLMCTL_CHECK(dq.scalar_type() == at::kBFloat16 && dq.sizes() == q.sizes() && dk.sizes() == k.sizes() &&
                   dv.sizes() == k.sizes() && delta.numel() == lse.numel(),
               "fa_bwd_ablate: bf16 dq/dk/dv, fp32 delta");
  const c10::DeviceGuard g(q.device());
  const double scale = 1.0 / std::sqrt((double)D);
  BwdArgs a = make_args(dout, q, k, v, lse, delta, dq, dk, dv, scale);
  if (abl == 5 || abl == 7) {
    LLMCTL_CHECK(dq.numel() * 2 >= (long)q.size(0) * k.size(2) * ((q.size(1) + KV_KB - 1) / KV_KB) * 64,
                 "fa_bwd_ablate: dq too small for the timeline");
    a.stamps = reinterpret_cast<unsigned long long*>(dq.data_ptr());
  }
  auto rck = row_consts(a, lse);
  if (abl == 1 || abl >= 3) {
    rck.narrow(0, 0, lse.numel()).copy_(lse.reshape(-1) * (-1.0 / scale));
    rck.narrow(0, lse.numel(), lse.numel()).copy_(-delta.reshape(-1));
  }
  dispatch_bwd(a, D, true, false, stream(), abl == 0 || abl == 2, abl != 2, abl >= 3 ? (int)abl - 3 : -1);
}

TORCH_LIBRARY_IMPL(llmctl, CUDA, m) {
  m.impl("flash_attn_bwd", &flash_attn_bwd);
  m.impl("flash_attn_bwd_qkv", &flash_attn_bwd_qkv);
  m.impl("fa_bwd_ablate", &fa_bwd_ablate);
}

}
```

### llmctl/ops/csrc/flash_attn_fwd.hip

```cpp
#include <cstdlib>

#include "attn_common.h"

namespace llmctl {
using namespace attn;
namespace {

constexpr int KB = 64;
constexpr float kRescaleTh = 8.f;

struct FwdArgs {
  const unsigned short* q;
  const unsigned short* k;
  const unsigned short* v;
  unsigned short* o;
  float* lse;
  int B, S, Hq, Hkv;
  long q_sb, q_ss, q_sh;
  long k_sb, k_ss, k_sh;
  long v_sb, v_ss, v_sh;
  long o_sb, o_ss, o_sh;
  float scale_log2;
  const int* doc;
  unsigned short* o_part;
  float* lse_part;
  int prio;
};

template <int HD, bool CAUSAL, bool DOC = false, bool SPLIT = false, int NW = 4, int NBUF = 2>
__global__ __launch_bounds__(NW * 64, 2) void fa_fwd_kernel(FwdArgs a) {
  constexpr int QB = NW * 32;
  constexpr int NTHR = NW * 64;
  constexpr int NKS = HD / 16;
  constexpr int NDB = HD / 32;
  constexpr int ROWB = HD * 2;
  constexpr int TILE = KB * ROWB;
  constexpr int PPW = TILE / 1024 / NW;
  constexpr int SLOT = 2 * TILE;
  static_assert(PPW * NW * 1024 == TILE, "pieces must split evenly over the waves");
  __shared__ __attribute__((aligned(1024))) unsigned char smem[NBUF * SLOT];

  const int tid = threadIdx.x;
  const int lane = tid & 63;
  const int wave = __builtin_amdgcn_readfirstlane(tid >> 6);
  const int r = lane & 31, hh = lane >> 5;
  const int nqb = (a.S + QB - 1) / QB;
  const int BH = a.B * a.Hq;
  int bh, rest;
  if (SPLIT || BH % 8) {
    bh = blockIdx.x % BH;
    rest = blockIdx.x / BH;
  } else {
    const int x = blockIdx.x & 7, j = blockIdx.x >> 3;
    bh = x * (BH >> 3) + j / nqb;
    rest = j % nqb;
  }
  const int part = SPLIT ? rest & 1 : 0;
  const int qblk = nqb - 1 - (SPLIT ? rest >> 1 : rest);
  const int b = bh / a.Hq, hq = bh % a.Hq;
  const int hk = hq / (a.Hq / a.Hkv);
  const int q_row0 = qblk * QB + wave * 32;
  const int my_q = q_row0 + r;

  const unsigned short* Qp = a.q + b * a.q_sb + hq * a.q_sh;
  const unsigned short* Kp = a.k + b * a.k_sb + hk * a.k_sh;
  const unsigned short* Vp = a.v + b * a.v_sb + hk * a.v_sh;

#pragma unroll
  for (int i = 0; i < NBUF * SLOT / (NTHR * 16); ++i)
    *reinterpret_cast<uint4*>(smem + i * NTHR * 16 + tid * 16) = make_uint4(0, 0, 0, 0);

  bf16x8_t qf[NKS];
#pragma unroll
  for (int ks = 0; ks < NKS; ++ks) {
    uint4 u = make_uint4(0, 0, 0, 0);
    if (my_q < a.S) u = gload16(Qp + (long)my_q * a.q_ss + ks * 16 + 8 * hh);
    qf[ks] = __builtin_bit_cast(bf16x8_t, u);
  }

  f32x16 o[NDB];
#pragma unroll
  for (int d = 0; d < NDB; ++d)
#pragma unroll
    for (int i = 0; i < 16; ++i) o[d][i] = 0.f;
  float m_i = -INFINITY, l_i = 0.f;

  const int kv_end = CAUSAL ? min(a.S, qblk * QB + QB) : a.S;
  int ntiles = (kv_end + KB - 1) / KB;
  int my_start = 0, w_min = 0, w_max = 0, t0 = 0;
  if constexpr (DOC) {
    const int* ds = a.doc + (long)b * a.S;
    my_start = ds[min(my_q, a.S - 1)];
    w_min = __builtin_amdgcn_readfirstlane(ds[min(q_row0, a.S - 1)]);
    w_max = __builtin_amdgcn_readfirstlane(ds[min(q_row0 + 31, a.S - 1)]);
    t0 = __builtin_amdgcn_readfirstlane(ds[min(qblk * QB, a.S - 1)]) / KB;
  }
  if constexpr (SPLIT) {
    const int mid = (t0 + ntiles) / 2;
    if (part == 0) ntiles = mid;
    else t0 = mid;
  }

  unsigned vk[PPW], vv[PPW];
#pragma unroll
  for (int i = 0; i < PPW; ++i) {
    const int byte = (i * NW + wave) * 1024 + lane * 16;
    const int row = byte / ROWB, pch = (byte % ROWB) >> 4;
    vk[i] = (unsigned)((row * a.k_ss + ((pch ^ swz_row<HD>(row)) << 3)) * 2);
    vv[i] = (unsigned)((row * a.v_ss + ((pch ^ swz_tr<HD>(row)) << 3)) * 2);
  }
  const unsigned lds0 = lds_addr(smem);
  int ik0 = t0 * KB;
  const unsigned short* kc = Kp + (long)ik0 * a.k_ss;
  const unsigned short* vc = Vp + (long)ik0 * a.v_ss;
  const long k_step = (long)KB * a.k_ss, v_step = (long)KB * a.v_ss;
  auto issue = [&](auto slot_c) __attribute__((always_inline)) {
    constexpr int SLC = decltype(slot_c)::value;
    const int nk = min(KB, a.S - ik0);
    i32x4_t rk = buf_rsrc(kc, (unsigned)(((nk - 1) * a.k_ss + HD) * 2));
    i32x4_t rv = buf_rsrc(vc, (unsigned)(((nk - 1) * a.v_ss + HD) * 2));
    asm volatile("s_nop 4" : "+s"(rk), "+s"(rv));
    const unsigned slot = lds0 + (unsigned)(SLC * SLOT) + wave * 1024;
#pragma unroll
    for (int i = 0; i < PPW; ++i) {
      buf_dma16(rk, vk[i], slot + i * NW * 1024);
      buf_dma16(rv, vv[i], slot + TILE + i * NW * 1024);
    }
    ik0 += KB;
    kc += k_step;
    vc += v_step;
  };

  const float c = a.scale_log2;
  const int key_hi = CAUSAL ? min(my_q, a.S - 1) : a.S - 1;
  int vlo[NDB], vhi[NDB];
#pragma unroll
  for (int d = 0; d < NDB; ++d) tr_frag_offs<HD>(d * 32, lane, vlo[d], vhi[d]);
  int kofs[NKS];
#pragma unroll
  for (int ks = 0; ks < NKS; ++ks) kofs[ks] = row_off<HD>(r, 2 * ks + hh);
#pragma unroll
  for (int ks = 0; ks < NKS; ++ks) asm volatile("" ::"v"(qf[ks]));
  auto tile = [&](bool need_mask, const unsigned char* Ks, const unsigned char* Vs, int kv0) __attribute__((always_inline)) {
    if (a.prio) __builtin_amdgcn_s_setprio(1);
    f32x16 s[2];
#pragma unroll
    for (int kb = 0; kb < 2; ++kb) {
#pragma unroll
      for (int i = 0; i < 16; ++i) s[kb][i] = 0.f;
#pragma unroll
      for (int ks = 0; ks < NKS; ++ks) s[kb] = mfma32(lds_read_b128(Ks, kb * 32 * (HD * 2) + kofs[ks]), qf[ks], s[kb]);
    }
    if (need_mask) {
#pragma unroll
      for (int kb = 0; kb < 2; ++kb)
#pragma unroll
        for (int i = 0; i < 16; ++i) {
          const int key = kv0 + kb * 32 + acc_row(i, hh);
          bool ok = key <= key_hi;
          if constexpr (DOC) ok = ok && key >= my_start;
          s[kb][i] = ok ? s[kb][i] : -INFINITY;
        }
    }
    if (a.prio) __builtin_amdgcn_s_setprio(0);
    float mx = s[0][0];
#pragma unroll
    for (int kb = 0; kb < 2; ++kb)
#pragma unroll
      for (int i = (kb == 0 ? 1 : 0); i < 16; ++i) mx = fmaxf(mx, s[kb][i]);
    mx = xor32_max(mx) * c;
    const bool grow = __builtin_amdgcn_ballot_w64(mx > m_i + kRescaleTh) != 0;
    const float m_new = grow ? fmaxf(m_i, mx) : m_i;
    const float nm = (m_new == -INFINITY) ? 0.f : -m_new;
    float rs = 0.f;
    bf16x8_t pb[2][2];
#pragma unroll
    for (int kb = 0; kb < 2; ++kb) {
      float p[16];
#pragma unroll
      for (int i = 0; i < 16; ++i) {
        p[i] = fast_exp2(__builtin_fmaf(s[kb][i], c, nm));
        rs += p[i];
      }
      pb[kb][0] = to_bf16x8(p);
      pb[kb][1] = to_bf16x8(p + 8);
    }
    rs = xor32_add(rs);
    if (grow) {
      const float alpha = fast_exp2(m_i + nm);
      l_i *= alpha;
#pragma unroll
      for (int d = 0; d < NDB; ++d)
#pragma unroll
        for (int i = 0; i < 16; ++i) o[d][i] *= alpha;
    }
    l_i += rs;
    m_i = m_new;
    if (a.prio) __builtin_amdgcn_s_setprio(1);
#pragma unroll
    for (int kb = 0; kb < 2; ++kb)
#pragma unroll
      for (int st = 0; st < 2; ++st)
#pragma unroll
        for (int d = 0; d < NDB; ++d) o[d] = mfma32(tr_frag_at<HD>(Vs, kb * 32 + 16 * st, vlo[d], vhi[d]), pb[kb][st], o[d]);
    if (a.prio) __builtin_amdgcn_s_setprio(0);
  };

  __syncthreads();
  auto step = [&](auto slot_c, int t) __attribute__((always_inline)) {
    constexpr int SL = decltype(slot_c)::value;
    if constexpr (NBUF == 3) {
      if (t + 1 < ntiles) vm_wait_n<2 * PPW>();
      else vm_wait_n<0>();
    } else {
      vm_wait_n<0>();
    }
    __builtin_amdgcn_s_barrier();
    if (t + NBUF - 1 < ntiles) issue(std::integral_constant<int, (SL + NBUF - 1) % NBUF>{});
    const int kv0 = t * KB;
    bool live = true;
    if constexpr (CAUSAL) live = kv0 <= q_row0 + 31;
    if constexpr (DOC) live = live && kv0 + KB > w_min;
    if (live) {
      const bool need_mask = (CAUSAL && kv0 + KB - 1 > q_row0) || (kv0 + KB > a.S) || (DOC && kv0 < w_max);
      tile(need_mask, smem + SL * SLOT, smem + SL * SLOT + TILE, kv0);
    }
  };
  if (t0 < ntiles) issue(std::integral_constant<int, 0>{});
  if constexpr (NBUF == 3)
    if (t0 + 1 < ntiles) issue(std::integral_constant<int, 1>{});
  for (int t = t0; t < ntiles; t += NBUF) {
    step(std::integral_constant<int, 0>{}, t);
    if (t + 1 < ntiles) step(std::integral_constant<int, 1>{}, t + 1);
    if constexpr (NBUF == 3)
      if (t + 2 < ntiles) step(std::integral_constant<int, 2>{}, t + 2);
  }

  if constexpr (SPLIT) {
    if (my_q < a.S) {
      const float inv = l_i > 0.f ? 1.f / l_i : 0.f;
      unsigned short* Op = a.o_part + ((((long)part * a.B + b) * a.S + my_q) * a.Hq + hq) * HD;
#pragma unroll
      for (int d = 0; d < NDB; ++d)
#pragma unroll
        for (int g = 0; g < 4; ++g) {
          const int col = d * 32 + 8 * g + 4 * hh;
          unsigned short w4[4];
#pragma unroll
          for (int j = 0; j < 4; ++j) w4[j] = f2bf(o[d][4 * g + j] * inv);
          *reinterpret_cast<uint2*>(Op + col) =
              make_uint2((unsigned)w4[0] | ((unsigned)w4[1] << 16), (unsigned)w4[2] | ((unsigned)w4[3] << 16));
        }
      if (hh == 0)
        a.lse_part[(((long)part * a.B + b) * a.Hq + hq) * a.S + my_q] =
            (l_i > 0.f) ? (m_i + __log2f(l_i)) * 0.69314718055994531f : -INFINITY;
    }
    return;
  }
  if (my_q < a.S) {
    const float inv = l_i > 0.f ? 1.f / l_i : 0.f;
    unsigned short* Op = a.o + b * a.o_sb + (long)my_q * a.o_ss + hq * a.o_sh;
#pragma unroll
    for (int d = 0; d < NDB; ++d)
#pragma unroll
      for (int g = 0; g < 4; ++g) {
        const int col = d * 32 + 8 * g + 4 * hh;
        unsigned short w4[4];
#pragma unroll
        for (int j = 0; j < 4; ++j) w4[j] = f2bf(o[d][4 * g + j] * inv);
        *reinterpret_cast<uint2*>(Op + col) =
            make_uint2((unsigned)w4[0] | ((unsigned)w4[1] << 16), (unsigned)w4[2] | ((unsigned)w4[3] << 16));
      }
    if (hh == 0) {
      const float lse = (l_i > 0.f) ? (m_i + __log2f(l_i)) * 0.69314718055994531f : -INFINITY;
      a.lse[((long)b * a.Hq + hq) * a.S + my_q] = lse;
    }
  }
}

template <int HD>
__global__ __launch_bounds__(256) void fa_combine_kernel(const unsigned short* __restrict__ o_part,
                                                         const float* __restrict__ lse_part,
                                                         unsigned short* __restrict__ o, float* __restrict__ lse,
                                                         int B, int S, int Hq, long o_sb, long o_ss, long o_sh) {
  constexpr int LPR = HD / 8;
  const long gid = (long)blockIdx.x * 256 + threadIdx.x;
  const long row = gid / LPR;
  const int sub = gid % LPR;
  if (row >= (long)B * S * Hq) return;
  const int hq = row % Hq;
  const long bs = row / Hq;
  const int sq = bs % S;
  const int b = bs / S;
  const long li = ((long)b * Hq + hq) * S + sq;
  const long plane = (long)B * Hq * S;
  const float l0 = lse_part[li], l1 = lse_part[plane + li];
  const float m = fmaxf(l0, l1);
  float w0 = 0.f, w1 = 0.f, l = -INFINITY;
  if (m != -INFINITY) {
    const float e0 = __expf(l0 - m), e1 = __expf(l1 - m);
    l = m + __logf(e0 + e1);
    w0 = e0 / (e0 + e1);
    w1 = e1 / (e0 + e1);
  }
  const long ob = row * HD + sub * 8;
  const long osz = (long)B * S * Hq * HD;
  float out[8], x0[8], x1[8];
  load8(o_part + ob, x0);
  load8(o_part + osz + ob, x1);
#pragma unroll
  for (int j = 0; j < 8; ++j) out[j] = w0 * x0[j] + w1 * x1[j];
  store8(o + b * o_sb + (long)sq * o_ss + (long)hq * o_sh + sub * 8, out);
  if (sub == 0) lse[li] = l;
}

template <int NW, int NBUF>
std::tuple<at::Tensor, at::Tensor> fwd_launch(const at::Tensor& q, at::Tensor& o, at::Tensor& lse, FwdArgs& a, int B,
                                              int S, int Hq, int D, bool causal,
                                              const c10::optional<at::Tensor>& doc_start) {
  constexpr int QB = NW * 32, WG_PER_CU = NW == 4 ? 2 : 1;
  const int nqb = (S + QB - 1) / QB;
  dim3 grid((unsigned)(B * Hq * nqb)), block(NW * 64);
  auto s = stream();
  bool split = causal && !(doc_start.has_value() && doc_start->defined()) && nqb >= 4 &&
               (long)B * Hq * nqb <= (long)WG_PER_CU * num_cus();
  if (const int64_t e = knob("fa_split", -1); e == 0) split = false;
  else if (e == 1) split = causal && !(doc_start.has_value() && doc_start->defined()) && nqb >= 2;
  if (split) {
    auto o_part = at::empty({2, B, S, Hq, D}, q.options());
    auto lse_part = at::empty({2, B, Hq, S}, q.options().dtype(at::kFloat));
    a.o_part = bf_mut(o_part);
    a.lse_part = lse_part.data_ptr<float>();
    dim3 g2((unsigned)(2 * B * Hq * nqb));
    const long threads = (long)B * S * Hq * (D / 8);
    if (D == 128) {
      hipLaunchKernelGGL((fa_fwd_kernel<128, true, false, true, NW, NBUF>), g2, block, 0, s, a);
      hipLaunchKernelGGL(fa_combine_kernel<128>, dim3((threads + 255) / 256), dim3(256), 0, s, a.o_part, a.lse_part,
                         bf_mut(o), lse.data_ptr<float>(), B, S, Hq, o.stride(0), o.stride(1), o.stride(2));
    } else {
      hipLaunchKernelGGL((fa_fwd_kernel<64, true, false, true, NW, NBUF>), g2, block, 0, s, a);
      hipLaunchKernelGGL(fa_combine_kernel<64>, dim3((threads + 255) / 256), dim3(256), 0, s, a.o_part, a.lse_part,
                         bf_mut(o), lse.data_ptr<float>(), B, S, Hq, o.stride(0), o.stride(1), o.stride(2));
    }
    return {o, lse};
  }
  if (doc_start.has_value() && doc_start->defined()) {
    const at::Tensor& ds = *doc_start;
    LLMCTL_CHECK(causal, "flash_attn_fwd: doc_start (packed sequences) needs causal attention");
    LLMCTL_CHECK(ds.is_cuda() && ds.scalar_type() == at::kInt && ds.is_contiguous() && ds.dim() == 2 &&
                     ds.size(0) == B && ds.size(1) == S,
                 "flash_attn_fwd: doc_start must be contiguous int32 [B,S]");
    a.doc = ds.data_ptr<int>();
    if (D == 128) hipLaunchKernelGGL((fa_fwd_kernel<128, true, true, false, NW, NBUF>), grid, block, 0, s, a);
    else hipLaunchKernelGGL((fa_fwd_kernel<64, true, true, false, NW, NBUF>), grid, block, 0, s, a);
    return {o, lse};
  }
  if (D == 128) {
    if (causal) hipLaunchKernelGGL((fa_fwd_kernel<128, true, false, false, NW, NBUF>), grid, block, 0, s, a);
    else hipLaunchKernelGGL((fa_fwd_kernel<128, false, false, false, NW, NBUF>), grid, block, 0, s, a);
  } else {
    if (causal) hipLaunchKernelGGL((fa_fwd_kernel<64, true, false, false, NW, NBUF>), grid, block, 0, s, a);
    else hipLaunchKernelGGL((fa_fwd_kernel<64, false, false, false, NW, NBUF>), grid, block, 0, s, a);
  }
  return {o, lse};
}

}

std::tuple<at::Tensor, at::Tensor> flash_attn_fwd(const at::Tensor& q, const at::Tensor& k, const at::Tensor& v,
                                                  double scale, bool causal,
                                                  const c10::optional<at::Tensor>& doc_start) {
  LLMCTL_CHECK(q.is_cuda() && k.is_cuda() && v.is_cuda(), "flash_attn_fwd: GPU tensors");
  LLMCTL_CHECK(q.scalar_type() == at::kBFloat16 && k.scalar_type() == at::kBFloat16 &&
                   v.scalar_type() == at::kBFloat16,
               "flash_attn_fwd: bf16");
  LLMCTL_CHECK(q.dim() == 4 && k.dim() == 4 && v.dim() == 4, "q/k/v must be [B,S,H,D]");
  const int B = q.size(0), S = q.size(1), Hq = q.size(2), D = q.size(3);
  const int Hkv = k.size(2);
  LLMCTL_CHECK(k.size(0) == B && k.size(1) == S && v.sizes() == k.sizes() && k.size(3) == D,
               "k/v shape must be [B,S,Hkv,D] matching q");
  LLMCTL_CHECK(Hq % Hkv == 0, "Hq must be a multiple of Hkv");
  LLMCTL_CHECK(D == 64 || D == 128, "head_dim must be 64 or 128, got ", D);
  LLMCTL_CHECK(q.stride(3) == 1 && k.stride(3) == 1 && v.stride(3) == 1, "head_dim must be contiguous");
  for (const at::Tensor* t : {&q, &k, &v})
    LLMCTL_CHECK(t->stride(0) % 8 == 0 && t->stride(1) % 8 == 0 && t->stride(2) % 8 == 0 &&
                     (reinterpret_cast<uintptr_t>(t->data_ptr()) & 15) == 0,
                 "q/k/v strides must be multiples of 8 elements and 16-B aligned");
  const c10::DeviceGuard g(q.device());
  auto o = at::empty({B, S, Hq, D}, q.options());
  auto lse = at::empty({B, Hq, S}, q.options().dtype(at::kFloat));
  if (B * S * Hq == 0) return {o, lse};
  FwdArgs a{bf_ptr(q), bf_ptr(k), bf_ptr(v), bf_mut(o), lse.data_ptr<float>(), B, S, Hq, Hkv,
            q.stride(0), q.stride(1), q.stride(2), k.stride(0), k.stride(1), k.stride(2),
            v.stride(0), v.stride(1), v.stride(2), o.stride(0), o.stride(1), o.stride(2),
            (float)(scale * 1.4426950408889634), nullptr, nullptr, nullptr, 0};
  a.prio = knob("fa_prio", 1) != 0 ? 1 : 0;
  if (knob("fa_nw", 4) == 8) return fwd_launch<8, 3>(q, o, lse, a, B, S, Hq, D, causal, doc_start);
  return fwd_launch<4, 2>(q, o, lse, a, B, S, Hq, D, causal, doc_start);
}

TORCH_LIBRARY_IMPL(llmctl, CUDA, m) { m.impl("flash_attn_fwd", &flash_attn_fwd); }

}
```

Before: 31050 tokens/s.

## Add lean flash-attention prologue and 16-byte paired output stores

Adds an fa_lean knob, on by default, for the forward and dq/dkv backward flash-attention kernels. With it set, the LDS ring zeroing is skipped when S is a multiple of the key block, and the first K/V tile load is issued before the Q/dO loads so the prologue overlaps with it. Output stores (O, dQ, dK, dV) use permlane32 swaps to pair lanes into 16-byte stores instead of 8-byte ones. The persistent dKV kernel also issues the next K/V load before the epilogue stores. The cost is more template variants and reliance on alignment checks plus the S-divisibility condition for correctness.

```diff
diff --git a/llmctl/config/knobs.py b/llmctl/config/knobs.py
--- a/llmctl/config/knobs.py
+++ b/llmctl/config/knobs.py
@@ -29,6 +29,7 @@
     fa_split: int = -1
     fa_prio: int = 1
     fa_nw: int = 4
+    fa_lean: int = 1
     dkv: int = 2
     dkv_nwg: int = 0
     async_tp: bool = True
@@ -51,7 +52,7 @@
         return dataclasses.asdict(self)
 
 
-NATIVE = ("fa_split", "fa_prio", "fa_nw", "dkv", "dkv_nwg", "decode_splits", "decode_v3")
+NATIVE = ("fa_split", "fa_prio", "fa_nw", "fa_lean", "dkv", "dkv_nwg", "decode_splits", "decode_v3")
 _FIELDS = {f.name: f for f in fields(PerfKnobs)}
 
 
diff --git a/llmctl/ops/csrc/attn_common.h b/llmctl/ops/csrc/attn_common.h
--- a/llmctl/ops/csrc/attn_common.h
+++ b/llmctl/ops/csrc/attn_common.h
@@ -23,6 +23,16 @@
 __device__ __forceinline__ float xor32_add(float x) {
   const auto r = __builtin_amdgcn_permlane32_swap(__float_as_uint(x), __float_as_uint(x), false, false);
   return __uint_as_float(r[0]) + __uint_as_float(r[1]);
+}
+
+__device__ __forceinline__ uint2 pack_bf16x4(const float* x) {
+  return make_uint2((unsigned)f2bf(x[0]) | ((unsigned)f2bf(x[1]) << 16),
+                    (unsigned)f2bf(x[2]) | ((unsigned)f2bf(x[3]) << 16));
+}
+__device__ __forceinline__ uint4 pair16(uint2 a, uint2 b) {
+  const auto x = __builtin_amdgcn_permlane32_swap(a.x, b.x, false, false);
+  const auto y = __builtin_amdgcn_permlane32_swap(a.y, b.y, false, false);
+  return make_uint4(x[0], y[0], x[1], y[1]);
 }
 
 __device__ __forceinline__ int acc_row(int i, int h) { return (i & 3) + 8 * (i >> 2) + 4 * h; }
diff --git a/llmctl/ops/csrc/flash_attn_bwd.hip b/llmctl/ops/csrc/flash_attn_bwd.hip
--- a/llmctl/ops/csrc/flash_attn_bwd.hip
+++ b/llmctl/ops/csrc/flash_attn_bwd.hip
@@ -39,6 +39,7 @@
   float* rck_w;
   long rc_n;
   unsigned long long* stamps = nullptr;
+  int lean = 0, wide = 0;
 };
 
 template <int NDB>
@@ -73,12 +74,12 @@
   }
 }
 
+__device__ __forceinline__ uint2 scaled_bf16x4(const float* x, float mul) {
+  const float y[4] = {x[0] * mul, x[1] * mul, x[2] * mul, x[3] * mul};
+  return pack_bf16x4(y);
+}
 __device__ __forceinline__ void store_bf16x4(unsigned short* p, const float* x, float mul) {
-  unsigned short w[4];
-#pragma unroll
-  for (int j = 0; j < 4; ++j) w[j] = f2bf(x[j] * mul);
-  *reinterpret_cast<uint2*>(p) =
-      make_uint2((unsigned)w[0] | ((unsigned)w[1] << 16), (unsigned)w[2] | ((unsigned)w[3] << 16));
+  *reinterpret_cast<uint2*>(p) = scaled_bf16x4(x, mul);
 }
 
 template <int HD, typename AccT>
@@ -116,6 +117,71 @@
       for (int j = 0; j < 4; ++j) x[j] = acc[d][4 * g + j];
       store_bf16x4(dst + d * 32 + 8 * g + 4 * hh, x, mul);
     }
+}
+
+template <int HD, typename AccT>
+__device__ __forceinline__ void store_row16(unsigned short* dst, const AccT* acc, float mul, int hh,
+                                            const float* cos_row, const float* sin_row, bool ok) {
+  constexpr int NDB = HD / 32;
+  unsigned short* p = dst + 8 * hh;
+  if (cos_row != nullptr) {
+    constexpr int HB = NDB / 2;
+#pragma unroll
+    for (int d = 0; d < HB; ++d)
+#pragma unroll
+      for (int g = 0; g < 4; g += 2) {
+        uint2 lo2[2], hi2[2];
+#pragma unroll
+        for (int e = 0; e < 2; ++e) {
+          const int c = d * 32 + 8 * (g + e) + 4 * hh;
+          const float4 cs = *reinterpret_cast<const float4*>(cos_row + c);
+          const float4 sn = *reinterpret_cast<const float4*>(sin_row + c);
+          const float cv[4] = {cs.x, cs.y, cs.z, cs.w}, sv[4] = {sn.x, sn.y, sn.z, sn.w};
+          float lo[4], hi[4];
+#pragma unroll
+          for (int j = 0; j < 4; ++j) {
+            const float x1 = acc[d][4 * (g + e) + j], x2 = acc[d + HB][4 * (g + e) + j];
+            lo[j] = x1 * cv[j] + x2 * sv[j];
+            hi[j] = x2 * cv[j] - x1 * sv[j];
+          }
+          lo2[e] = scaled_bf16x4(lo, mul);
+          hi2[e] = scaled_bf16x4(hi, mul);
+        }
+        const uint4 wl = pair16(lo2[0], lo2[1]), wh = pair16(hi2[0], hi2[1]);
+        if (ok) {
+          *reinterpret_cast<uint4*>(p + d * 32 + 8 * g) = wl;
+          *reinterpret_cast<uint4*>(p + d * 32 + 8 * g + HD / 2) = wh;
+        }
+      }
+    return;
+  }
+#pragma unroll
+  for (int d = 0; d < NDB; ++d)
+#pragma unroll
+    for (int g = 0; g < 4; g += 2) {
+      float x[8];
+#pragma unroll
+      for (int j = 0; j < 8; ++j) x[j] = acc[d][4 * g + j];
+      const uint4 w = pair16(scaled_bf16x4(x, mul), scaled_bf16x4(x + 4, mul));
+      if (ok) *reinterpret_cast<uint4*>(p + d * 32 + 8 * g) = w;
+    }
+}
+
+template <int HD, typename AccT>
+__device__ __forceinline__ void store_out_row(const BwdArgs& a, unsigned short* out, long st, int b, int row,
+                                              int head, const AccT* acc, float mul, int hh, bool rope) {
+  const bool ok = row < a.S;
+  if (!a.wide && !ok) return;
+  const long tok = (long)b * a.S + min(row, a.S - 1);
+  const float *cr = nullptr, *sr = nullptr;
+  if (rope && a.cos_t != nullptr) {
+    const long p = a.rope_pos ? (long)a.rope_pos[tok] : tok % a.rope_S;
+    cr = a.cos_t + p * (HD / 2);
+    sr = a.sin_t + p * (HD / 2);
+  }
+  unsigned short* dst = out + tok * st + (long)head * HD;
+  if (a.wide) store_row16<HD>(dst, acc, mul, hh, cr, sr, ok);
+  else store_row<HD>(dst, acc, mul, hh, cr, sr);
 }
 
 template <int HD, bool CAUSAL, bool DOC>
@@ -352,19 +418,8 @@
   }
 #pragma unroll
   for (int d = 0; d < NDB; ++d) asm volatile("s_nop 7\n\ts_nop 7" : "+a"(dk[d]), "+a"(dv[d]));
-  if (my_key < a.S) {
-    const long tok = (long)b * a.S + my_key;
-    unsigned short* dkp = a.dk + tok * a.dk_st + (long)hk * HD;
-    unsigned short* dvp = a.dv + tok * a.dv_st + (long)hk * HD;
-    const float *cr = nullptr, *sr = nullptr;
-    if (a.cos_t != nullptr) {
-      const long p = a.rope_pos ? (long)a.rope_pos[tok] : tok % a.rope_S;
-      cr = a.cos_t + p * (HD / 2);
-      sr = a.sin_t + p * (HD / 2);
-    }
-    store_row<HD>(dkp, dk, a.scale, hh, cr, sr);
-    store_row<HD>(dvp, dv, 1.f, hh, nullptr, nullptr);
-  }
+  store_out_row<HD>(a, a.dk, a.dk_st, b, my_key, hk, dk, a.scale, hh, true);
+  store_out_row<HD>(a, a.dv, a.dv_st, b, my_key, hk, dv, 1.f, hh, false);
 }
 
 using s2_t = __attribute__((ext_vector_type(2))) unsigned int;
@@ -686,19 +741,8 @@
   stamp(3);
 #pragma unroll
   for (int d = 0; d < NDB; ++d) asm volatile("s_nop 7\n\ts_nop 7" : "+a"(dk[d]), "+a"(dv[d]));
-  if (my_key < a.S) {
-    const long tok = (long)b * a.S + my_key;
-    unsigned short* dkp = a.dk + tok * a.dk_st + (long)hk * HD;
-    unsigned short* dvp = a.dv + tok * a.dv_st + (long)hk * HD;
-    const float *cr = nullptr, *sr = nullptr;
-    if (a.cos_t != nullptr) {
-      const long p = a.rope_pos ? (long)a.rope_pos[tok] : tok % a.rope_S;
-      cr = a.cos_t + p * (HD / 2);
-      sr = a.sin_t + p * (HD / 2);
-    }
-    store_row<HD>(dkp, dk, a.scale, hh, cr, sr);
-    store_row<HD>(dvp, dv, 1.f, hh, nullptr, nullptr);
-  }
+  store_out_row<HD>(a, a.dk, a.dk_st, b, my_key, hk, dk, a.scale, hh, true);
+  store_out_row<HD>(a, a.dv, a.dv_st, b, my_key, hk, dv, 1.f, hh, false);
   if constexpr (STAMP) {
     asm volatile("s_waitcnt vmcnt(0)" ::: "memory");
     __syncthreads();
@@ -707,7 +751,7 @@
   }
 }
 
-template <bool STAMP>
+template <bool STAMP, bool WIDE>
 __global__ __launch_bounds__(256, 1) void fa_bwd_dkv_persist_kernel(BwdArgs a, int* __restrict__ wq) {
   constexpr int HD = 128;
   constexpr int NKS = HD / 16;
@@ -956,7 +1000,7 @@
       unsigned short* dkp = a.dk + tok * a.dk_st + (long)hk * HD;
       unsigned short* dvp = a.dv + tok * a.dv_st + (long)hk * HD;
       const bool rope = a.cos_t != nullptr;
-      f32x4 cs[NDB / 2][4], sn[NDB / 2][4];
+      f32x4 cs[NDB / 2][4] = {}, sn[NDB / 2][4] = {};
       if (rope) {
         const long p = a.rope_pos ? (long)a.rope_pos[tok] : tok % a.rope_S;
         const float* cr = a.cos_t + p * (HD / 2);
@@ -978,43 +1022,94 @@
         w[1] = (unsigned)f2bf(x[2] * mul) | ((unsigned)f2bf(x[3] * mul) << 16);
         asm volatile("global_store_dwordx2 %0, %1, off" ::"v"(p), "v"(w) : "memory");
       };
-#pragma unroll
-      for (int d = 0; d < NDB / 2; ++d) {
-        const f32x16 x1 = acc_copy(dk[d]), x2 = acc_copy(dk[d + NDB / 2]);
-        acc_zero(dk[d]);
-        acc_zero(dk[d + NDB / 2]);
-#pragma unroll
-        for (int g = 0; g < 4; ++g) {
-          const int col = d * 32 + 8 * g + 4 * hh;
-          float lo[4], hi[4];
-#pragma unroll
-          for (int j = 0; j < 4; ++j) {
-            const float c1 = rope ? cs[d][g][j] : 1.f, s1 = rope ? sn[d][g][j] : 0.f;
-            lo[j] = x1[4 * g + j] * c1 + x2[4 * g + j] * s1;
-            hi[j] = x2[4 * g + j] * c1 - x1[4 * g + j] * s1;
+      auto st16 = [&](unsigned short* p, uint2 w0, uint2 w1) __attribute__((always_inline)) {
+        using u4 = __attribute__((ext_vector_type(4))) unsigned;
+        const uint4 t = pair16(w0, w1);
+        const u4 w = {t.x, t.y, t.z, t.w};
+        asm volatile("global_store_dwordx4 %0, %1, off\n\ts_nop 1" ::"v"(p), "v"(w) : "memory");
+      };
+      if constexpr (WIDE) {
+#pragma unroll
+        for (int d = 0; d < NDB / 2; ++d)
+#pragma unroll
+          for (int g = 0; g < 4; ++g) asm volatile("" ::"v"(cs[d][g]), "v"(sn[d][g]));
+        load_kv(pend0 >= 0 ? pend0 : cur);
+#pragma unroll
+        for (int d = 0; d < NDB / 2; ++d) {
+          const f32x16 x1 = acc_copy(dk[d]), x2 = acc_copy(dk[d + NDB / 2]);
+          acc_zero(dk[d]);
+          acc_zero(dk[d + NDB / 2]);
+#pragma unroll
+          for (int g = 0; g < 4; g += 2) {
+            uint2 lo2[2], hi2[2];
+#pragma unroll
+            for (int e = 0; e < 2; ++e) {
+              float lo[4], hi[4];
+#pragma unroll
+              for (int j = 0; j < 4; ++j) {
+                const float c1 = rope ? cs[d][g + e][j] : 1.f, s1 = rope ? sn[d][g + e][j] : 0.f;
+                lo[j] = x1[4 * (g + e) + j] * c1 + x2[4 * (g + e) + j] * s1;
+                hi[j] = x2[4 * (g + e) + j] * c1 - x1[4 * (g + e) + j] * s1;
+              }
+              lo2[e] = scaled_bf16x4(lo, a.scale);
+              hi2[e] = scaled_bf16x4(hi, a.scale);
+            }
+            const int col = d * 32 + 8 * g + 8 * hh;
+            st16(dkp + col, lo2[0], lo2[1]);
+            st16(dkp + col + HD / 2, hi2[0], hi2[1]);
           }
-          st8(dkp + col, lo, a.scale);
-          st8(dkp + col + HD / 2, hi, a.scale);
         }
-      }
-#pragma unroll
-      for (int d = 0; d < NDB; ++d) {
-        const f32x16 x = acc_copy(dv[d]);
-        acc_zero(dv[d]);
-#pragma unroll
-        for (int g = 0; g < 4; ++g) {
-          float y[4];
-#pragma unroll
-          for (int j = 0; j < 4; ++j) y[j] = x[4 * g + j];
-          st8(dvp + d * 32 + 8 * g + 4 * hh, y, 1.f);
+#pragma unroll
+        for (int d = 0; d < NDB; ++d) {
+          const f32x16 x = acc_copy(dv[d]);
+          acc_zero(dv[d]);
+#pragma unroll
+          for (int g = 0; g < 4; g += 2) {
+            float y[8];
+#pragma unroll
+            for (int j = 0; j < 8; ++j) y[j] = x[4 * g + j];
+            st16(dvp + d * 32 + 8 * g + 8 * hh, scaled_bf16x4(y, 1.f), scaled_bf16x4(y + 4, 1.f));
+          }
         }
-      }
-      load_kv(pend0 >= 0 ? pend0 : cur);
-      asm volatile("s_waitcnt vmcnt(0)"
+      } else {
+#pragma unroll
+        for (int d = 0; d < NDB / 2; ++d) {
+          const f32x16 x1 = acc_copy(dk[d]), x2 = acc_copy(dk[d + NDB / 2]);
+          acc_zero(dk[d]);
+          acc_zero(dk[d + NDB / 2]);
+#pragma unroll
+          for (int g = 0; g < 4; ++g) {
+            const int col = d * 32 + 8 * g + 4 * hh;
+            float lo[4], hi[4];
+#pragma unroll
+            for (int j = 0; j < 4; ++j) {
+              const float c1 = rope ? cs[d][g][j] : 1.f, s1 = rope ? sn[d][g][j] : 0.f;
+              lo[j] = x1[4 * g + j] * c1 + x2[4 * g + j] * s1;
+              hi[j] = x2[4 * g + j] * c1 - x1[4 * g + j] * s1;
+            }
+            st8(dkp + col, lo, a.scale);
+            st8(dkp + col + HD / 2, hi, a.scale);
+          }
+        }
+#pragma unroll
+        for (int d = 0; d < NDB; ++d) {
+          const f32x16 x = acc_copy(dv[d]);
+          acc_zero(dv[d]);
+#pragma unroll
+          for (int g = 0; g < 4; ++g) {
+            float y[4];
+#pragma unroll
+            for (int j = 0; j < 4; ++j) y[j] = x[4 * g + j];
+            st8(dvp + d * 32 + 8 * g + 4 * hh, y, 1.f);
+          }
+        }
+      }
+      if constexpr (!WIDE) load_kv(pend0 >= 0 ? pend0 : cur);
+      asm volatile("s_waitcnt vmcnt(%16)"
                    : "+a"(kf[0]), "+a"(kf[1]), "+a"(kf[2]), "+a"(kf[3]), "+a"(kf[4]), "+a"(kf[5]), "+a"(kf[6]),
                      "+a"(kf[7]), "+a"(vf[0]), "+a"(vf[1]), "+a"(vf[2]), "+a"(vf[3]), "+a"(vf[4]), "+a"(vf[5]),
                      "+a"(vf[6]), "+a"(vf[7])
-                   :
+                   : "i"(WIDE ? 16 : 0)
                    : "memory");
     }
     stamp(2);
@@ -1062,50 +1157,12 @@
   const unsigned short* Kp = a.k + b * a.k_sb + hk * a.k_sh;
   const unsigned short* Vp = a.v + b * a.v_sb + hk * a.v_sh;
 
-#pragma unroll
-  for (int i = 0; i < 2 * SLOT / 4096; ++i)
-    *reinterpret_cast<uint4*>(smem + i * 4096 + tid * 16) = make_uint4(0, 0, 0, 0);
-
-  bf16x8_t qf[NKS], df[NKS];
-  {
-    const unsigned short* Qp = a.q + b * a.q_sb + hq * a.q_sh + (long)qc * a.q_ss + 8 * hh;
-    const unsigned short* Dp = a.dout + b * a.do_sb + hq * a.do_sh + (long)qc * a.do_ss + 8 * hh;
-#pragma unroll
-    for (int ks = 0; ks < NKS; ++ks) {
-      qf[ks] = __builtin_bit_cast(bf16x8_t, gload16(Qp + 16 * ks));
-      df[ks] = __builtin_bit_cast(bf16x8_t, gload16(Dp + 16 * ks));
-    }
-  }
-  const long rc = ((long)b * a.Hq + hq) * a.S + qc;
-  const float nlse2 = -a.lse[rc] * LOG2E;
-  float dlt;
-  if (a.o != nullptr) {
-    const unsigned short* Op = a.o + b * a.o_sb + hq * a.o_sh + (long)qc * a.o_ss + 8 * hh;
-    float acc = 0.f;
-#pragma unroll
-    for (int ks = 0; ks < NKS; ++ks) {
-      const bf16x8_t of = __builtin_bit_cast(bf16x8_t, gload16(Op + 16 * ks));
-#pragma unroll
-      for (int j = 0; j < 8; ++j) acc += (float)of[j] * (float)df[ks][j];
-    }
-    dlt = xor32_add(acc);
-    if (hh == 0 && my_q < a.S) a.delta_w[rc] = dlt;
-  } else {
-    dlt = a.delta[rc];
-  }
-  if (hh == 0 && my_q < a.S) {
-    a.rck_w[rc] = -a.lse[rc] / a.scale;
-    a.rck_w[a.rc_n + rc] = -dlt;
-  }
-#pragma unroll
-  for (int ks = 0; ks < NKS; ++ks) asm volatile("" ::"v"(qf[ks]), "v"(df[ks]));
-  asm volatile("" ::"v"(nlse2), "v"(dlt));
-
-  f32x16 dq[NDB];
-#pragma unroll
-  for (int d = 0; d < NDB; ++d)
-#pragma unroll
-    for (int i = 0; i < 16; ++i) dq[d][i] = 0.f;
+  const bool zero_ring = !a.lean || a.S % DQ_KB != 0;
+  if (zero_ring) {
+#pragma unroll
+    for (int i = 0; i < 2 * SLOT / 4096; ++i)
+      *reinterpret_cast<uint4*>(smem + i * 4096 + tid * 16) = make_uint4(0, 0, 0, 0);
+  }
 
   const int kv_end = CAUSAL ? min(a.S, qblk * DQ_QB + DQ_QB) : a.S;
   const int ntiles = (kv_end + DQ_KB - 1) / DQ_KB;
@@ -1158,6 +1215,52 @@
     vc += v_step;
   };
 
+  if (a.lean) {
+    if (zero_ring) __syncthreads();
+    if (t0 < ntiles) issue(std::integral_constant<int, 0>{});
+  }
+
+  bf16x8_t qf[NKS], df[NKS];
+  {
+    const unsigned short* Qp = a.q + b * a.q_sb + hq * a.q_sh + (long)qc * a.q_ss + 8 * hh;
+    const unsigned short* Dp = a.dout + b * a.do_sb + hq * a.do_sh + (long)qc * a.do_ss + 8 * hh;
+#pragma unroll
+    for (int ks = 0; ks < NKS; ++ks) {
+      qf[ks] = __builtin_bit_cast(bf16x8_t, gload16(Qp + 16 * ks));
+      df[ks] = __builtin_bit_cast(bf16x8_t, gload16(Dp + 16 * ks));
+    }
+  }
+  const long rc = ((long)b * a.Hq + hq) * a.S + qc;
+  const float nlse2 = -a.lse[rc] * LOG2E;
+  float dlt;
+  if (a.o != nullptr) {
+    const unsigned short* Op = a.o + b * a.o_sb + hq * a.o_sh + (long)qc * a.o_ss + 8 * hh;
+    float acc = 0.f;
+#pragma unroll
+    for (int ks = 0; ks < NKS; ++ks) {
+      const bf16x8_t of = __builtin_bit_cast(bf16x8_t, gload16(Op + 16 * ks));
+#pragma unroll
+      for (int j = 0; j < 8; ++j) acc += (float)of[j] * (float)df[ks][j];
+    }
+    dlt = xor32_add(acc);
+    if (hh == 0 && my_q < a.S) a.delta_w[rc] = dlt;
+  } else {
+    dlt = a.delta[rc];
+  }
+  if (hh == 0 && my_q < a.S) {
+    a.rck_w[rc] = -a.lse[rc] / a.scale;
+    a.rck_w[a.rc_n + rc] = -dlt;
+  }
+#pragma unroll
+  for (int ks = 0; ks < NKS; ++ks) asm volatile("" ::"v"(qf[ks]), "v"(df[ks]));
+  asm volatile("" ::"v"(nlse2), "v"(dlt));
+
+  f32x16 dq[NDB];
+#pragma unroll
+  for (int d = 0; d < NDB; ++d)
+#pragma unroll
+    for (int i = 0; i < 16; ++i) dq[d][i] = 0.f;
+
   auto tile = [&](bool need_mask, const unsigned char* Ks, const unsigned char* Vs, int kv0)
                   __attribute__((always_inline)) {
 #pragma unroll
@@ -1191,7 +1294,7 @@
     }
   };
 
-  __syncthreads();
+  if (!a.lean) __syncthreads();
   auto step = [&](auto slot_c, int t) __attribute__((always_inline)) {
     constexpr int SL = decltype(slot_c)::value;
     vm_wait_n<0>();
@@ -1207,21 +1310,12 @@
       tile(need_mask, smem + SL * SLOT, smem + SL * SLOT + TILE, kv0);
     }
   };
-  if (t0 < ntiles) issue(std::integral_constant<int, 0>{});
+  if (!a.lean && t0 < ntiles) issue(std::integral_constant<int, 0>{});
   for (int t = t0; t < ntiles; t += 2) {
     step(std::integral_constant<int, 0>{}, t);
     if (t + 1 < ntiles) step(std::integral_constant<int, 1>{}, t + 1);
   }
-  if (my_q < a.S) {
-    const long tok = (long)b * a.S + my_q;
-    const float *cr = nullptr, *sr = nullptr;
-    if (a.cos_t != nullptr) {
-      const long p = a.rope_pos ? (long)a.rope_pos[tok] : tok % a.rope_S;
-      cr = a.cos_t + p * (HD / 2);
-      sr = a.sin_t + p * (HD / 2);
-    }
-    store_row<HD>(a.dq + tok * a.dq_st + (long)hq * HD, dq, a.scale, hh, cr, sr);
-  }
+  store_out_row<HD>(a, a.dq, a.dq_st, b, my_q, hq, dq, a.scale, hh, true);
 }
 
 int dkv_mode() {
@@ -1262,10 +1356,9 @@
           const int min_wg = ((long)a.B * a.Hkv) % 8 == 0 ? 8 : 1;
           if (const int64_t e = knob("dkv_nwg", 0); e > 0) nwg = std::max<int>(min_wg, std::min<int>(nwg, (int)e));
           nwg = std::max(nwg, min_wg);
-          if (a.stamps != nullptr)
-            hipLaunchKernelGGL(fa_bwd_dkv_persist_kernel<true>, dim3((unsigned)nwg), dim3(256), 0, s, a, wq);
-          else
-            hipLaunchKernelGGL(fa_bwd_dkv_persist_kernel<false>, dim3((unsigned)nwg), dim3(256), 0, s, a, wq);
+          auto kern = a.stamps != nullptr ? (a.wide ? fa_bwd_dkv_persist_kernel<true, true> : fa_bwd_dkv_persist_kernel<true, false>)
+                                          : (a.wide ? fa_bwd_dkv_persist_kernel<false, true> : fa_bwd_dkv_persist_kernel<false, false>);
+          hipLaunchKernelGGL(kern, dim3((unsigned)nwg), dim3(256), 0, s, a, wq);
           return;
         }
       }
@@ -1278,8 +1371,14 @@
   }
 }
 
-void dispatch_bwd(const BwdArgs& a, int D, bool causal, bool doc, hipStream_t s, bool do_dq = true,
+void dispatch_bwd(const BwdArgs& a0, int D, bool causal, bool doc, hipStream_t s, bool do_dq = true,
                   bool do_dkv = true, int dkv_impl = -1) {
+  BwdArgs a = a0;
+  a.lean = knob("fa_lean", 1) != 0 ? 1 : 0;
+  bool al = true;
+  for (const unsigned short* p : {a.dq, a.dk, a.dv}) al = al && (reinterpret_cast<uintptr_t>(p) & 15) == 0;
+  for (const long st : {a.dq_st, a.dk_st, a.dv_st}) al = al && st % 8 == 0;
+  a.wide = a.lean && al ? 1 : 0;
   if (doc) {
     if (D == 128) launch_bwd<128, true, true>(a, s, do_dq, do_dkv, dkv_impl);
     else launch_bwd<64, true, true>(a, s, do_dq, do_dkv, dkv_impl);
diff --git a/llmctl/ops/csrc/flash_attn_fwd.hip b/llmctl/ops/csrc/flash_attn_fwd.hip
--- a/llmctl/ops/csrc/flash_attn_fwd.hip
+++ b/llmctl/ops/csrc/flash_attn_fwd.hip
@@ -25,6 +25,7 @@
   unsigned short* o_part;
   float* lse_part;
   int prio;
+  int lean;
 };
 
 template <int HD, bool CAUSAL, bool DOC = false, bool SPLIT = false, int NW = 4, int NBUF = 2>
@@ -66,24 +67,12 @@
   const unsigned short* Kp = a.k + b * a.k_sb + hk * a.k_sh;
   const unsigned short* Vp = a.v + b * a.v_sb + hk * a.v_sh;
 
-#pragma unroll
-  for (int i = 0; i < NBUF * SLOT / (NTHR * 16); ++i)
-    *reinterpret_cast<uint4*>(smem + i * NTHR * 16 + tid * 16) = make_uint4(0, 0, 0, 0);
-
-  bf16x8_t qf[NKS];
-#pragma unroll
-  for (int ks = 0; ks < NKS; ++ks) {
-    uint4 u = make_uint4(0, 0, 0, 0);
-    if (my_q < a.S) u = gload16(Qp + (long)my_q * a.q_ss + ks * 16 + 8 * hh);
-    qf[ks] = __builtin_bit_cast(bf16x8_t, u);
-  }
-
-  f32x16 o[NDB];
-#pragma unroll
-  for (int d = 0; d < NDB; ++d)
-#pragma unroll
-    for (int i = 0; i < 16; ++i) o[d][i] = 0.f;
-  float m_i = -INFINITY, l_i = 0.f;
+  const bool zero_ring = !a.lean || a.S % KB != 0;
+  if (zero_ring) {
+#pragma unroll
+    for (int i = 0; i < NBUF * SLOT / (NTHR * 16); ++i)
+      *reinterpret_cast<uint4*>(smem + i * NTHR * 16 + tid * 16) = make_uint4(0, 0, 0, 0);
+  }
 
   const int kv_end = CAUSAL ? min(a.S, qblk * QB + QB) : a.S;
   int ntiles = (kv_end + KB - 1) / KB;
@@ -130,6 +119,30 @@
     kc += k_step;
     vc += v_step;
   };
+  auto first_issue = [&]() __attribute__((always_inline)) {
+    if (t0 < ntiles) issue(std::integral_constant<int, 0>{});
+    if constexpr (NBUF == 3)
+      if (t0 + 1 < ntiles) issue(std::integral_constant<int, 1>{});
+  };
+  if (a.lean) {
+    if (zero_ring) __syncthreads();
+    first_issue();
+  }
+
+  bf16x8_t qf[NKS];
+#pragma unroll
+  for (int ks = 0; ks < NKS; ++ks) {
+    uint4 u = make_uint4(0, 0, 0, 0);
+    if (my_q < a.S) u = gload16(Qp + (long)my_q * a.q_ss + ks * 16 + 8 * hh);
+    qf[ks] = __builtin_bit_cast(bf16x8_t, u);
+  }
+
+  f32x16 o[NDB];
+#pragma unroll
+  for (int d = 0; d < NDB; ++d)
+#pragma unroll
+    for (int i = 0; i < 16; ++i) o[d][i] = 0.f;
+  float m_i = -INFINITY, l_i = 0.f;
 
   const float c = a.scale_log2;
   const int key_hi = CAUSAL ? min(my_q, a.S - 1) : a.S - 1;
@@ -206,7 +219,7 @@
     if (a.prio) __builtin_amdgcn_s_setprio(0);
   };
 
-  __syncthreads();
+  if (!a.lean) __syncthreads();
   auto step = [&](auto slot_c, int t) __attribute__((always_inline)) {
     constexpr int SL = decltype(slot_c)::value;
     if constexpr (NBUF == 3) {
@@ -226,9 +239,7 @@
       tile(need_mask, smem + SL * SLOT, smem + SL * SLOT + TILE, kv0);
     }
   };
-  if (t0 < ntiles) issue(std::integral_constant<int, 0>{});
-  if constexpr (NBUF == 3)
-    if (t0 + 1 < ntiles) issue(std::integral_constant<int, 1>{});
+  if (!a.lean) first_issue();
   for (int t = t0; t < ntiles; t += NBUF) {
     step(std::integral_constant<int, 0>{}, t);
     if (t + 1 < ntiles) step(std::integral_constant<int, 1>{}, t + 1);
@@ -236,46 +247,41 @@
       if (t + 2 < ntiles) step(std::integral_constant<int, 2>{}, t + 2);
   }
 
+  auto store_o = [&](unsigned short* Op, float inv) __attribute__((always_inline)) {
+    if (a.lean) {
+      const bool ok = my_q < a.S;
+#pragma unroll
+      for (int d = 0; d < NDB; ++d)
+#pragma unroll
+        for (int g = 0; g < 4; g += 2) {
+          float x[8];
+#pragma unroll
+          for (int j = 0; j < 8; ++j) x[j] = o[d][4 * g + j] * inv;
+          const uint4 w = pair16(pack_bf16x4(x), pack_bf16x4(x + 4));
+          if (ok) *reinterpret_cast<uint4*>(Op + d * 32 + 8 * g + 8 * hh) = w;
+        }
+      return;
+    }
+    if (my_q >= a.S) return;
+#pragma unroll
+    for (int d = 0; d < NDB; ++d)
+#pragma unroll
+      for (int g = 0; g < 4; ++g) {
+        float x[4];
+#pragma unroll
+        for (int j = 0; j < 4; ++j) x[j] = o[d][4 * g + j] * inv;
+        *reinterpret_cast<uint2*>(Op + d * 32 + 8 * g + 4 * hh) = pack_bf16x4(x);
+      }
+  };
+  const float inv = l_i > 0.f ? 1.f / l_i : 0.f;
+  const float lse = (l_i > 0.f) ? (m_i + __log2f(l_i)) * 0.69314718055994531f : -INFINITY;
   if constexpr (SPLIT) {
-    if (my_q < a.S) {
-      const float inv = l_i > 0.f ? 1.f / l_i : 0.f;
-      unsigned short* Op = a.o_part + ((((long)part * a.B + b) * a.S + my_q) * a.Hq + hq) * HD;
-#pragma unroll
-      for (int d = 0; d < NDB; ++d)
-#pragma unroll
-        for (int g = 0; g < 4; ++g) {
-          const int col = d * 32 + 8 * g + 4 * hh;
-          unsigned short w4[4];
-#pragma unroll
-          for (int j = 0; j < 4; ++j) w4[j] = f2bf(o[d][4 * g + j] * inv);
-          *reinterpret_cast<uint2*>(Op + col) =
-              make_uint2((unsigned)w4[0] | ((unsigned)w4[1] << 16), (unsigned)w4[2] | ((unsigned)w4[3] << 16));
-        }
-      if (hh == 0)
-        a.lse_part[(((long)part * a.B + b) * a.Hq + hq) * a.S + my_q] =
-            (l_i > 0.f) ? (m_i + __log2f(l_i)) * 0.69314718055994531f : -INFINITY;
-    }
+    store_o(a.o_part + ((((long)part * a.B + b) * a.S + my_q) * a.Hq + hq) * HD, inv);
+    if (hh == 0 && my_q < a.S) a.lse_part[(((long)part * a.B + b) * a.Hq + hq) * a.S + my_q] = lse;
     return;
   }
-  if (my_q < a.S) {
-    const float inv = l_i > 0.f ? 1.f / l_i : 0.f;
-    unsigned short* Op = a.o + b * a.o_sb + (long)my_q * a.o_ss + hq * a.o_sh;
-#pragma unroll
-    for (int d = 0; d < NDB; ++d)
-#pragma unroll
-      for (int g = 0; g < 4; ++g) {
-        const int col = d * 32 + 8 * g + 4 * hh;
-        unsigned short w4[4];
-#pragma unroll
-        for (int j = 0; j < 4; ++j) w4[j] = f2bf(o[d][4 * g + j] * inv);
-        *reinterpret_cast<uint2*>(Op + col) =
-            make_uint2((unsigned)w4[0] | ((unsigned)w4[1] << 16), (unsigned)w4[2] | ((unsigned)w4[3] << 16));
-      }
-    if (hh == 0) {
-      const float lse = (l_i > 0.f) ? (m_i + __log2f(l_i)) * 0.69314718055994531f : -INFINITY;
-      a.lse[((long)b * a.Hq + hq) * a.S + my_q] = lse;
-    }
-  }
+  store_o(a.o + b * a.o_sb + (long)my_q * a.o_ss + hq * a.o_sh, inv);
+  if (hh == 0 && my_q < a.S) a.lse[((long)b * a.Hq + hq) * a.S + my_q] = lse;
 }
 
 template <int HD>
@@ -393,8 +399,9 @@
   FwdArgs a{bf_ptr(q), bf_ptr(k), bf_ptr(v), bf_mut(o), lse.data_ptr<float>(), B, S, Hq, Hkv,
             q.stride(0), q.stride(1), q.stride(2), k.stride(0), k.stride(1), k.stride(2),
             v.stride(0), v.stride(1), v.stride(2), o.stride(0), o.stride(1), o.stride(2),
-            (float)(scale * 1.4426950408889634), nullptr, nullptr, nullptr, 0};
+            (float)(scale * 1.4426950408889634), nullptr, nullptr, nullptr, 0, 0};
   a.prio = knob("fa_prio", 1) != 0 ? 1 : 0;
+  a.lean = knob("fa_lean", 1) != 0 ? 1 : 0;
   if (knob("fa_nw", 4) == 8) return fwd_launch<8, 3>(q, o, lse, a, B, S, Hq, D, causal, doc_start);
   return fwd_launch<4, 2>(q, o, lse, a, B, S, Hq, D, causal, doc_start);
 }
```

Result: no change. 31200 tokens/s, median of 6 (+0.5%).
